# morisUtokyo/mTR

Measured on AMD Instinct MI355X. Metric: reads/sec, 2 kb Nanopore synthetic, higher is better.
Workload: dtype int32

## Files before the change

### mtr_amd/csrc/device_util.hip.inc

```
#pragma once
#include <hip/hip_runtime.h>
#include "mtr_common.h"
#include "walk_screen.h"

#define DEVINL __device__ __forceinline__

typedef __attribute__((address_space(3))) int lds_int;
typedef __attribute__((address_space(3))) unsigned char lds_u8;

DEVINL int lane_id() { return (int)(threadIdx.x & 63u); }
__device__ long long mtr_dev_wrap_dp_size = MTRC_WRAP_DP_SIZE;
DEVINL bool dp_size_ok(int U, int rows) { return (size_t)(U + 1) * (size_t)rows + (size_t)U < (size_t)mtr_dev_wrap_dp_size; }
DEVINL int uni(int v) { return __builtin_amdgcn_readfirstlane(v); }
DEVINL long long uni64(long long v)
{
    const unsigned lo = (unsigned)__builtin_amdgcn_readfirstlane((int)(unsigned)v);
    const unsigned hi = (unsigned)__builtin_amdgcn_readfirstlane((int)(unsigned)((unsigned long long)v >> 32));
    return (long long)(((unsigned long long)hi << 32) | lo);
}
DEVINL int bcast(int v, int src) { return __shfl(v, src, 64); }
DEVINL unsigned long long lanemask_lt() { return (1ull << lane_id()) - 1ull; }
DEVINL int mbcnt(unsigned long long m)
{
    return (int)__builtin_amdgcn_mbcnt_hi((unsigned)(m >> 32), __builtin_amdgcn_mbcnt_lo((unsigned)m, 0u));
}
DEVINL int first_lane(unsigned long long m) { return __ffsll((long long)m) - 1; }


DEVINL unsigned scan_max_u32(unsigned v);
DEVINL int wave_max_i32(int v)
{
    for (int d = 32; d > 0; d >>= 1) { int o = __shfl_xor(v, d, 64); v = o > v ? o : v; }
    return v;
}
DEVINL int lane_val(int v, int l) { return __builtin_amdgcn_readlane(v, l); }
DEVINL int write_lane(int v, int val, int l)
{
    asm("s_mov_b32 m0, %2\n\tv_writelane_b32 %0, %1, m0" : "+v"(v) : "s"(val), "s"(l) : "m0");
    return v;
}
DEVINL void write_lane2(int &a, int &b, int va, int vb, int l)
{
    asm("s_mov_b32 m0, %4\n\tv_writelane_b32 %0, %2, m0\n\tv_writelane_b32 %1, %3, m0" : "+v"(a), "+v"(b) : "s"(va), "s"(vb), "s"(l & 63) : "m0");
}
DEVINL long long lane_val64(long long v, int l)
{
    const unsigned lo = (unsigned)__builtin_amdgcn_readlane((int)(unsigned)v, l), hi = (unsigned)__builtin_amdgcn_readlane((int)(unsigned)((unsigned long long)v >> 32), l);
    return (long long)(((unsigned long long)hi << 32) | lo);
}
DEVINL int wave_max_i32_dpp(int v) { return lane_val((int)scan_max_u32((unsigned)(v + 1)), 63) - 1; }
DEVINL long long wave_sum_i64(long long v)
{
    for (int d = 32; d > 0; d >>= 1) v += __shfl_xor(v, d, 64);
    return v;
}

DEVINL unsigned scan_max_u32(unsigned v)
{
    unsigned t;
    t = (unsigned)__builtin_amdgcn_update_dpp(0, (int)v, 0x111, 0xf, 0xf, false); v = t > v ? t : v;
    t = (unsigned)__builtin_amdgcn_update_dpp(0, (int)v, 0x112, 0xf, 0xf, false); v = t > v ? t : v;
    t = (unsigned)__builtin_amdgcn_update_dpp(0, (int)v, 0x114, 0xf, 0xf, false); v = t > v ? t : v;
    t = (unsigned)__builtin_amdgcn_update_dpp(0, (int)v, 0x118, 0xf, 0xf, false); v = t > v ? t : v;
    t = (unsigned)__builtin_amdgcn_update_dpp(0, (int)v, 0x142, 0xa, 0xf, false); v = t > v ? t : v;
    t = (unsigned)__builtin_amdgcn_update_dpp(0, (int)v, 0x143, 0xc, 0xf, false); v = t > v ? t : v;
    return v;
}
DEVINL void scan_max_u32_x2(unsigned &a, unsigned &b)
{
    unsigned s, t;
#define MTR_SCAN_STEP(ctrl, rm) \
    s = (unsigned)__builtin_amdgcn_update_dpp(0, (int)a, ctrl, rm, 0xf, false); \
    t = (unsigned)__builtin_amdgcn_update_dpp(0, (int)b, ctrl, rm, 0xf, false); \
    a = s > a ? s : a; b = t > b ? t : b;
    MTR_SCAN_STEP(0x111, 0xf) MTR_SCAN_STEP(0x112, 0xf) MTR_SCAN_STEP(0x114, 0xf) MTR_SCAN_STEP(0x118, 0xf)
    MTR_SCAN_STEP(0x142, 0xa) MTR_SCAN_STEP(0x143, 0xc)
#undef MTR_SCAN_STEP
}
DEVINL void scan_max_u32_x2_row16(unsigned &a, unsigned &b)
{
    unsigned s, t;
#define MTR_SCAN_STEP(ctrl) \
    s = (unsigned)__builtin_amdgcn_update_dpp(0, (int)a, ctrl, 0xf, 0xf, false); \
    t = (unsigned)__builtin_amdgcn_update_dpp(0, (int)b, ctrl, 0xf, 0xf, false); \
    a = s > a ? s : a; b = t > b ? t : b;
    MTR_SCAN_STEP(0x111) MTR_SCAN_STEP(0x112) MTR_SCAN_STEP(0x114) MTR_SCAN_STEP(0x118)
#undef MTR_SCAN_STEP
}
DEVINL int row_shift_up1(int v, int first)
{
    return __builtin_amdgcn_update_dpp(first, v, 0x111, 0xf, 0xf, false);
}
typedef unsigned short u16x2 __attribute__((ext_vector_type(2)));
DEVINL u16x2 as_pk(unsigned v) { return __builtin_bit_cast(u16x2, v); }
DEVINL unsigned as_u32(u16x2 v) { return __builtin_bit_cast(unsigned, v); }
DEVINL unsigned pk_add(unsigned a, unsigned b) { return as_u32(as_pk(a) + as_pk(b)); }
DEVINL unsigned pk_sub(unsigned a, unsigned b) { return as_u32(as_pk(a) - as_pk(b)); }
DEVINL unsigned pk_sub_sat(unsigned a, unsigned b) { return as_u32(__builtin_elementwise_sub_sat(as_pk(a), as_pk(b))); }
DEVINL unsigned max3_u32(unsigned a, unsigned b, unsigned c) { unsigned r; asm("v_max3_u32 %0, %1, %2, %3" : "=v"(r) : "v"(a), "v"(b), "v"(c)); return r; }
DEVINL unsigned pk_max(unsigned a, unsigned b) { return as_u32(__builtin_elementwise_max(as_pk(a), as_pk(b))); }
DEVINL unsigned pk_min(unsigned a, unsigned b) { return as_u32(__builtin_elementwise_min(as_pk(a), as_pk(b))); }
template <int SH>
DEVINL unsigned lshl_or(unsigned a, unsigned b)
{
    unsigned r;
    asm("v_lshl_or_b32 %0, %1, %2, %3" : "=v"(r) : "v"(a), "n"(SH), "v"(b));
    return r;
}
DEVINL unsigned pk_nonzero(unsigned a, unsigned one_pk)
{
    unsigned r;
    asm("v_pk_min_u16 %0, %1, %2" : "=v"(r) : "v"(a), "v"(one_pk));
    return r;
}

DEVINL int shift_up1(int v, int first)
{
    return __builtin_amdgcn_update_dpp(first, v, 0x138, 0xf, 0xf, false);
}

DEVINL void scan_max_first(double &v, int &idx)
{
    int lane = lane_id();
    for (int d = 1; d < 64; d <<= 1) {
        double ov = __shfl_up(v, d, 64); int oi = __shfl_up(idx, d, 64);
        if (lane >= d && !(v > ov)) { v = ov; idx = oi; }
    }
}
DEVINL void scan_min_first(double &v, int &idx)
{
    int lane = lane_id();
    for (int d = 1; d < 64; d <<= 1) {
        double ov = __shfl_up(v, d, 64); int oi = __shfl_up(idx, d, 64);
        if (lane >= d && !(v < ov)) { v = ov; idx = oi; }
    }
}
// ... 134 lines not shown
```

### mtr_amd/csrc/dp_test.hip.inc

```
#pragma once
#include "dp_wrap.hip.inc"

struct DpPassArgs {
    DpTestArgs t;
    int32_t pass, n_groups;
    const int32_t *group_off;
    long long packed_words;
};

DEVINL void dpt_clear(DpRes &o) { o.stop_i = 0; o.end_i = 0; o.mat = o.mis = o.ins = o.del = o.scanned = 0; o.end_j = 0; }
DEVINL void dpt_store(const DpPassArgs &a, int task, int p, int qs, int U, const DpRes &o)
{
    if (lane_id() == 0) {
        int32_t *r = a.t.out8 + ((size_t)task * 2 + (size_t)p) * 8;
        r[0] = qs + o.stop_i + 1; r[1] = qs + o.end_i; r[2] = o.end_i - o.stop_i; r[3] = U > 0 ? o.scanned / U : 0;
        r[4] = o.mat; r[5] = o.mis; r[6] = o.ins; r[7] = o.del;
    }
}
template <int FMT>
DEVINL void dpt_traceback(const DpPassArgs &a, const uint32_t *pk, int qs, int U, const uint8_t *cells, int psel, int rstride, const int (&best)[3],
                          DpRes &o, unsigned long long *wc)
{
    dpt_clear(o);
    const int bv = uni(best[0]), bi = uni(best[1]), bj = uni(best[2]);
// ... 125 lines not shown
        }
        const int maxrows = uni(wave_max_i32(q.rows)), umax = uni(wave_max_i32(q.U));
        const int C = (umax + 7) >> 3;
        int best[2][3];
        st_fwd2p_oct(C, q, cells, maxrows, best);
        wave_sync_mem();
        const int bestl = st_oct_best_lanes(best);
#pragma unroll 1
        for (int g = 0; g < n; g++) {
            const int tg = t0 + g;
            const int rd = uni(a.t.read_idx[tg]), qs = uni(a.t.qs[tg]), U = uni(a.t.unit_off[tg + 1]) - uni(a.t.unit_off[tg]);
            for (int p = 0; p < 2; p++) {
                const int bk[3] = { lane_val(bestl, 8 * g + 3 * p), lane_val(bestl, 8 * g + 3 * p + 1), lane_val(bestl, 8 * g + 3 * p + 2) };
                DpRes o;
                dpt_traceback<1>(a, a.t.b.packed + uni64(a.t.b.woff[rd]), qs, U, cells + (size_t)g * DPQ_DP_BYTES_G(8, C, maxrows), p, DPQ_ROW_BYTES_G(8, C), bk, o, s_cnt);
                dpt_store(a, tg, p, qs, U, o);
                loop_join();
            }
            loop_join();
        }
        wave_sync_mem();
        loop_join();
    }
    wc_flush(s_cnt, a.t.counters);
}

__global__ __launch_bounds__(64, MTR_WAVES_PER_SIMD) void mtr_k_dp_test_rev(DpPassArgs a)
{
    __shared__ unsigned long long s_cnt[CNT_N];
    if (lane_id() < CNT_N) s_cnt[lane_id()] = 0ull;
    uint8_t *cells = a.t.scratch + (size_t)blockIdx.x * a.t.scratch_per_wave;
    for (;;) {
        const int grp = next_work_item(a.t.work_counter);
        if (grp >= a.n_groups) break;
        const int t0 = uni(a.group_off[grp]), n = uni(a.group_off[grp + 1]) - t0;
        DpOct q; q.n = n;
        int maxrows = 0, maxU = 0;
#pragma unroll 1
        for (int g = 0; g < RQ_SLOTS; g++) { q.pk[g] = a.t.b.packed; q.wlim[g] = 1; q.base[g] = 0; q.rows[g] = 0; q.U[g] = 0; q.unit[g] = cells; q.G[g] = 1; q.MM[g] = 1; q.D[g] = 1; }
#pragma unroll 1
        for (int k = 0; k < n; k++) {
            const int tg = t0 + k;
            const int rd = uni(a.t.read_idx[tg]), uo = uni(a.t.unit_off[tg]);
            q.pk[k] = a.t.b.packed + uni64(a.t.b.woff[rd]); q.wlim[k] = a.packed_words - uni64(a.t.b.woff[rd]);
            q.base[k] = uni(a.t.qs[tg]); q.rows[k] = uni(a.t.qe[tg]) - q.base[k] + 1;
            q.U[k] = uni(a.t.unit_off[tg + 1]) - uo; q.unit[k] = a.t.units + uo;
            q.G[k] = uni(a.t.gain[tg]); q.MM[k] = uni(a.t.mism[tg]); q.D[k] = uni(a.t.indel[tg]);
            maxrows = q.rows[k] > maxrows ? q.rows[k] : maxrows; maxU = q.U[k] > maxU ? q.U[k] : maxU;
        }
        const int Cq = DPQ_COLS(maxU);
        int best[RQ_SLOTS][3];
        for (int g = 0; g < RQ_SLOTS; g++) { best[g][0] = 0; best[g][1] = 0; best[g][2] = 0; }
        if (a.pass == MTR_TEST_PASS_FOUR1P) st_fwd1p_four(Cq, q, cells, maxrows, best); else st_fwd1p_any(Cq, q, cells, maxrows, best);
        wave_sync_mem();
#pragma unroll 1
        for (int k = 0; k < n; k++) {
            int bk[3] = { best[0][0], best[0][1], best[0][2] };
#pragma unroll
            for (int h = 1; h < RQ_SLOTS; h++) if (k == h) { bk[0] = best[h][0]; bk[1] = best[h][1]; bk[2] = best[h][2]; }
            const int tg = t0 + k;
            const int rd = uni(a.t.read_idx[tg]), qs = uni(a.t.qs[tg]), U = uni(a.t.unit_off[tg + 1]) - uni(a.t.unit_off[tg]);
            DpRes o;
            dpt_traceback<3>(a, a.t.b.packed + uni64(a.t.b.woff[rd]), qs, U, cells + (size_t)k * DPQP_DP_BYTES(Cq, maxrows), 0, DPQ_ROW_BYTES(Cq), bk, o, s_cnt);
            dpt_store(a, tg, 0, qs, U, o);
            loop_join();
        }
        wave_sync_mem();
        loop_join();
    }
    wc_flush(s_cnt, a.t.counters);
}

struct PolishTestArgs {
    K2Args a;
    int32_t n_tasks;
    const int32_t *read_idx, *rep_start, *rep_end, *k;
    const uint8_t *units; const int32_t *scores, *unit_off;
    uint8_t *out_units; int32_t *out_len;
};
__global__ __launch_bounds__(64, MTR_LAT_WAVES_PER_SIMD) void mtr_k_polish_test(PolishTestArgs p)
{
    __shared__ __attribute__((aligned(16))) int s_arena[MTR_ARENA_INTS];
    __shared__ unsigned long long s_cnt[CNT_N];
    int *s_keys = s_arena, *s_seeds = s_arena + K2_TAB_CAP, *s_stage = s_seeds + MTRC_MAX_SEEDS + 4;
    const int lane = lane_id();
    if (lane < CNT_N) s_cnt[lane] = 0ull;
    K2Ctx c;
    c.a = &p.a; c.wc = s_cnt;
    c.sc = p.a.scratch + (size_t)blockIdx.x * p.a.scratch_per_wave;
    c.y = k2_layout(p.a.Lmax, p.a.cells_cap);
    c.lds_keys = (lds_int *)s_keys; c.seeds = (lds_int *)s_seeds; c.stage = (lds_int *)s_stage;
    c.ties = (int *)(c.sc + c.y.ties); c.fresh = c.ties + MTRC_MAX_TIEBREAKS;
    c.memo_n = 0; c.memo_qs = c.memo_qe = -1; c.memo_U = 0; c.rmemo_n = 0;
    for (;;) {
        const int t = next_work_item(p.a.work_counter);
        if (t >= p.n_tasks) break;
        st_member_ctx(c, p.a, uni(p.read_idx[t]));
        const int uo = uni(p.unit_off[t]), U = uni(p.unit_off[t + 1]) - uo;
        RR r; rr_clear(r);
        r.rep_start = uni(p.rep_start[t]); r.rep_end = uni(p.rep_end[t]); r.kmer = uni(p.k[t]); r.period = U;
        uint8_t *ub = slot_unit(c, 1);
        slot_load_candidate(ub, slot_score(c, 1), p.units + uo, p.scores + uo, U);
        wave_sync_mem();
        polish(c, r, 1);
#pragma unroll 1
        for (int q = lane; q < r.period; q += 64) p.out_units[(size_t)t * MTRC_MAX_PERIOD + q] = ub[q];
        if (lane == 0) p.out_len[t] = r.period;
        wave_sync_mem();
        loop_join();
    }
    wc_flush(s_cnt, p.a.counters);
}

struct ReviseTestArgs {
    K2Args a;
    int32_t n_groups;
    const int32_t *group_off, *read_idx, *rr;
    const uint8_t *units; const int32_t *scores, *unit_off;
    int32_t *out_rr; uint8_t *out_units;
};
__global__ __launch_bounds__(64, MTR_WAVES_PER_SIMD) void mtr_k_revise_test(ReviseTestArgs p)
{
    __shared__ __attribute__((aligned(16))) int s_arena[MTR_ARENA_INTS];
    __shared__ unsigned long long s_cnt[CNT_N];
    int *s_keys = s_arena, *s_seeds = s_arena + K2_TAB_CAP, *s_stage = s_seeds + MTRC_MAX_SEEDS + 4;
    const int lane = lane_id();
    if (lane < CNT_N) s_cnt[lane] = 0ull;
    K2Ctx c;
    c.a = &p.a; c.wc = s_cnt;
    c.sc = p.a.scratch + (size_t)blockIdx.x * p.a.scratch_per_wave;
    c.y = k2_layout(p.a.Lmax, p.a.cells_cap);
    c.lds_keys = (lds_int *)s_keys; c.seeds = (lds_int *)s_seeds; c.stage = (lds_int *)s_stage;
    c.ties = (int *)(c.sc + c.y.ties); c.fresh = c.ties + MTRC_MAX_TIEBREAKS;
    for (;;) {
        const int grp = next_work_item(p.a.work_counter);
        if (grp >= p.n_groups) break;
        const int t0 = uni(p.group_off[grp]), t1 = uni(p.group_off[grp + 1]);
        c.memo_n = 0; c.memo_qs = c.memo_qe = -1; c.memo_U = 0; c.rmemo_n = 0;
#pragma unroll 1
        for (int t = t0; t < t1; t++) {
            st_member_ctx(c, p.a, uni(p.read_idx[t]));
            const int uo = uni(p.unit_off[t]), U = uni(p.unit_off[t + 1]) - uo;
            RR cur; st_rr_load(p.rr + (size_t)t * 13, cur);
            uint8_t *ub = slot_unit(c, 1);
            slot_load_candidate(ub, slot_score(c, 1), p.units + uo, p.scores + uo, U);
            wave_sync_mem();
            revise(c, cur);
            if (lane == 0) {
                int32_t *o = p.out_rr + (size_t)t * 13;
                o[0] = cur.rep_start; o[1] = cur.rep_end; o[2] = cur.repeat_len; o[3] = cur.period; o[4] = cur.copies; o[5] = cur.mat; o[6] = cur.mis;
                o[7] = cur.ins; o[8] = cur.del; o[9] = cur.kmer; o[10] = cur.G; o[11] = cur.MM; o[12] = cur.D;
            }
#pragma unroll 1
            for (int q = lane; q < cur.period && q < MTRC_MAX_PERIOD; q += 64) p.out_units[(size_t)t * MTRC_MAX_PERIOD + q] = ub[q];
            wave_sync_mem();
            loop_join();
        }
        loop_join();
    }
    wc_flush(s_cnt, p.a.counters);
}
```

### mtr_amd/csrc/k1_ranges.hip.inc

```
#pragma once
#include "device_util.hip.inc"


struct K1Pass { int k, w; };
typedef short k1_num;
static_assert(2 * MTRC_MAX_WINDOW <= 32767, "numerators in 16 bits");

DEVINL int k1_raw(const uint32_t *pk, const uint8_t *mt, int L, int r, int N, int idx)
{
    if (idx < r) return mt[N + idx];
    if (idx < r + L) return base_at(pk, idx - r);
    if (idx < L + 2 * r) return mt[N + r + (idx - r - L)];
    if (idx < N) return mt[idx];
    return 0;
}
DEVINL int k1_raw_tail(const uint32_t *pk, const uint8_t *mt, int L, int r, int N, int idx, const uint16_t *tail, int E, int tlen)
{
    if (idx >= E) return idx - E < tlen ? (int)tail[idx - E] : 0;
    return k1_raw(pk, mt, L, r, N, idx);
}

template <bool MANHATTAN>
DEVINL void k1_passes(const K1Layout &y, uint8_t *sc, unsigned short *hist, int hist_cap, int L, int r, int npass, int pass_k, int pass_w,
                      int32_t *status, int row_base = 0, int alloc_nb = 0)
// ... 1063 lines not shown
    }
    double *DI = (double *)(sc + y.di); int *END = (int *)(sc + y.end); int *W = (int *)(sc + y.w);
    if (parts & K1_CODES) for (int idx = lane; idx < n; idx += 64) DI[idx] = -1.0;
    wave_sync_mem();

    const bool rows_hold_d = MANHATTAN && (parts & K1_PASSES) && (parts & K1_FINISH) && only_pass < 0 && seg < 0 && !(MAY_FILE_ORDER && tlen > 0) && 2 * n <= arena_bytes;
    if (npass > 0 && (parts & K1_PASSES)) {
        const unsigned long long t_p = clk();
        int run_n = npass, run_k = my_k, run_w = my_w, row_base = 0;
        if (only_pass >= 0) {
            run_n = only_pass < npass ? 1 : 0; row_base = only_pass;
            run_k = __shfl(my_k, only_pass & 63, 64); run_w = __shfl(my_w, only_pass & 63, 64);
        }
        if (run_n > 0) {
            if (seg > 0 && MAY_FILE_ORDER && tlen > 0) {  }
            else if (seg >= 0 && !(MAY_FILE_ORDER && tlen > 0)) {
                if (MANHATTAN) k1_passes_manhattan(y, sc, arena, arena_bytes, L, r, 1, run_k, run_w, a.status, row_base, seg);
                else k1_pass_pearson_seg(y, sc, arena, L, r, run_k, run_w, only_pass, seg);
            }
            else if (MAY_FILE_ORDER && tlen > 0) k1_passes<MANHATTAN>(y, sc, (unsigned short *)arena, arena_bytes / 2, L, r, run_n, run_k, run_w, a.status, row_base, 1024);
            else if (MANHATTAN) k1_passes_manhattan(y, sc, arena, arena_bytes, L, r, run_n, run_k, run_w, a.status, row_base, -1, !rows_hold_d);
            else k1_passes<false>(y, sc, (unsigned short *)arena, arena_bytes / 2, L, r, run_n, run_k, run_w, a.status, row_base);
        }
        wc_time(wc, CYC_K1_PASSES, t_p);
    }
    if (!(parts & K1_FINISH)) return;
    if (npass > 0) {
        const unsigned long long t_e = clk();
        const double *tmp = (const double *)(sc + y.tmp);
        if (!(parts & K1_NO_EXTRACT))
        for (int p = 0; p < npass; p++) {
            int w = __shfl(my_w, p, 64);
            if (MANHATTAN) {
                const k1_num *row = (const k1_num *)(sc + y.tmp) + (size_t)p * n;
                if (2 * n <= arena_bytes) {
                    lds_i16 *r16 = (lds_i16 *)arena;
                    const int bits_at = (2 * n + 3) & ~3, bits_words = (n + 31) >> 5;
                    const bool bits = bits_at + 4 * bits_words <= arena_bytes;
                    lds_u32b *pres = (lds_u32b *)(arena + bits_at);
                    if (bits && p == 0) { for (int t = lane; t < bits_words; t += 64) pres[t] = 0u; }
                    if (rows_hold_d) {
                        const int ns = n - w - r - __shfl(my_k, p, 64) + 1;
                        for (int t = lane; t < n; t += 64) r16[t] = (short)((ns > 0 && t >= w && t < w + ns) ? (int)row[t - w] - (int)row[t] : -2 * w);
                    } else
                    for (int t = lane; t < n; t += 64) r16[t] = (short)row[t];
                    wave_sync_mem();
                    if (bits) k1_extract_int<true, true>(row, r16, n, w, DI, END, W, wc, pres); else k1_extract_int<true>(row, r16, n, w, DI, END, W, wc);
                    wave_sync_mem();
                } else k1_extract_int<false>(row, nullptr, n, w, DI, END, W, wc);
            }
            else k1_extract(tmp + (size_t)p * n, n, w, DI, END, W, wc);
        }
        wc_time(wc, CYC_K1_EXTRACT, t_e);
        wc_add(wc, CNT_DI_PASSES, npass);
        long long pos = (lane < npass) ? (long long)(n - my_w - r - my_k + 1) : 0; if (pos < 0) pos = 0;
        pos = wave_sum_i64(pos);
        wc_add(wc, CNT_DI_POS, pos);
    }

    const unsigned long long t_d = clk();
    int alive_n = 0;
    for (int base = 0; base < L; base += 64) {
        const int i = base + lane;
        alive_n += __popcll(__ballot(i < L && DI[i + r] != -1.0));
    }
    int nout;
    if ((alive_n + 1) * 20 <= arena_bytes) {
        lds_f64 *ld = (lds_f64 *)arena;
        lds_i32 *lp = (lds_i32 *)(arena + 8 * (alive_n + 1)), *le = lp + (alive_n + 1), *lw = le + (alive_n + 1);
        nout = k1_lists(a, rd, L, r, DI, END, W, lp, le, lw, ld, alive_n + 1);
    } else {
        int *lp = (int *)(sc + y.l_pos), *le = (int *)(sc + y.l_end), *lw = (int *)(sc + y.l_w);
        double *ld = (double *)(sc + y.l_di);
        nout = k1_lists(a, rd, L, r, DI, END, W, lp, le, lw, ld, y.cap);
    }
    const int ocap = mtrc_range_cap(L);
    if (nout > ocap) { set_status(a.status, DEV_ERR_RANGE_OVERFLOW); nout = ocap; }
    if (lane == 0) a.r_count[rd] = nout;
    wc_add(wc, CNT_RANGES_CAND, nout);
    wc_time(wc, CYC_K1_DEDUP, t_d);
    wc_time(wc, CYC_K1_TOTAL, t_start);
}

#define MTR_ARENA_INTS (2048 + 104 + 256)

__global__ __launch_bounds__(64, 4) void mtr_k1_part(K1Args a, int parts, const int32_t *item_read, const int32_t *item_pass, int n_items)
{
    __shared__ __attribute__((aligned(16))) int s_arena[MTR_ARENA_INTS];
    __shared__ unsigned long long s_cnt[CNT_N];
    if (lane_id() < CNT_N) s_cnt[lane_id()] = 0ull;
    for (;;) {
        const int t = next_work_item(a.work_counter);
        if (t >= n_items) break;
        const int rd = item_read ? __builtin_amdgcn_readfirstlane(item_read[t]) : t;
        const int pv = item_pass ? __builtin_amdgcn_readfirstlane(item_pass[t]) : -1;
        const int ps = pv < 0 ? -1 : (pv & 255), seg = pv < 0 ? -1 : (pv >> 8) - 1;
        uint8_t *sc = a.scratch + (size_t)rd * a.scratch_per_wave;
        if (a.manhattan) k1_read<true, true>(a, rd, sc, (lds_u8 *)s_arena, MTR_ARENA_INTS * 4, s_cnt, parts, ps, seg);
        else k1_read<false, true>(a, rd, sc, (lds_u8 *)s_arena, MTR_ARENA_INTS * 4, s_cnt, parts, ps, seg);
        loop_join();
    }
    wc_flush(s_cnt, a.counters);
}

#define K1_PIPE_ARENA_BYTES (K1_PIPE_WAVES * K1_TILE * 16)
__global__ __launch_bounds__(64 * K1_PIPE_WAVES) void mtr_k1_finish_pipe(K1Args a, int n_items, int seg_rows )
{
    __shared__ __attribute__((aligned(16))) int s_arena[K1_PIPE_ARENA_BYTES / 4];
    __shared__ unsigned long long s_cnt[K1_PIPE_WAVES][CNT_N];
    __shared__ int s_progress[MTRC_MAX_PASSES + 1];
    __shared__ int s_wg[2 * K1_PIPE_WAVES + 2];
    __shared__ int s_item;
#ifdef MTR_K1_COUNT
    __shared__ unsigned long long s_dbg[MTRC_MAX_PASSES + 1][5];
#endif
    const int wv = threadIdx.x >> 6, lane = lane_id();
    if (lane < CNT_N) s_cnt[wv][lane] = 0ull;
    for (;;) {
        __syncthreads();
        if (threadIdx.x == 0) s_item = (int)atomicAdd(a.work_counter, 1u);
        if (threadIdx.x < MTRC_MAX_PASSES + 1) s_progress[threadIdx.x] = 0;
        __syncthreads();
        const int rd = __builtin_amdgcn_readfirstlane(s_item);
        if (rd >= n_items) break;
        uint8_t *sc = a.scratch + (size_t)rd * a.scratch_per_wave;
        const int L = a.b.lens[rd];
        const int r = mtrc_rand_len(L);
        const int n = L + 2 * r;
        const K1Layout y = k1_layout(a.Lmax);
        double *DI = (double *)(sc + y.di); int *END = (int *)(sc + y.end); int *W = (int *)(sc + y.w);
        int npass = 0;
        for (int k = 1; k <= 5; k += 2) {
            const int max_w = (k == 1) ? 20 : (k == 3 ? 80 : MTRC_MAX_WINDOW);
            for (int w = MTRC_MIN_WINDOW; w <= max_w && w < L / 2; w *= 2) npass++;
        }
#ifdef MTR_K1_COUNT
        const unsigned long long tk0 = __builtin_amdgcn_s_memtime();
#endif
        for (int p = wv; p < npass; p += K1_PIPE_WAVES) {
            int w = 0, kk = 1, q = 0;
            for (int k = 1; k <= 5; k += 2) {
                const int max_w = (k == 1) ? 20 : (k == 3 ? 80 : MTRC_MAX_WINDOW);
                for (int ww = MTRC_MIN_WINDOW; ww <= max_w && ww < L / 2; ww *= 2) { if (q == p) { w = ww; kk = k; } q++; }
            }
            if (a.manhattan && seg_rows) { k1_numerators(y, sc, L, r, kk, w, p); wave_sync_mem(); }
            K1Pipe pp;
            pp.prev = p > 0 ? (volatile lds_i32 *)&s_progress[p - 1] : nullptr;
            pp.mine = (volatile lds_i32 *)&s_progress[p];
            lds_u8 *mine = (lds_u8 *)s_arena + (size_t)wv * (K1_TILE * 16);
            if (a.manhattan) {
                K1Tile<int, k1_num> tl; tl.val = (lds_i32 *)(mine + K1_TILE * 8); tl.di = (lds_f64 *)mine;
                tl.row = (const k1_num *)(sc + y.tmp) + (size_t)p * n; tl.DI = DI; tl.n = n; tl.t0 = 0; tl.tn = 0; tl.pad = 0; tl.pp = pp;
#ifdef MTR_K1_COUNT
                const unsigned long long tp0 = __builtin_amdgcn_s_memtime();
#endif
                k1_extract_int_tile(tl, n, w, DI, END, W, s_cnt[wv]);
#ifdef MTR_K1_COUNT
                if (lane == 0) { s_dbg[p][0] = tp0 - tk0; s_dbg[p][1] = __builtin_amdgcn_s_memtime() - tk0; s_dbg[p][2] = tl.c_wait; s_dbg[p][3] = tl.c_fill;
                                 s_dbg[p][4] = (unsigned long long)tl.n_rec | ((unsigned long long)tl.n_refill << 32); }
#endif
            } else {
                K1Tile<double> tl; tl.val = (lds_f64 *)(mine + K1_TILE * 8); tl.di = (lds_f64 *)mine;
                tl.row = (const double *)(sc + y.tmp) + (size_t)p * n; tl.DI = DI; tl.n = n; tl.t0 = 0; tl.tn = 0; tl.pad = 0.0; tl.pp = pp;
                k1_extract_tile(tl, n, w, DI, END, W);
            }
            wave_sync_mem();
            if (lane == 0) s_progress[p] = 0x7fffffff;
            loop_join();
        }
        __syncthreads();
#ifdef MTR_K1_COUNT
        const unsigned long long tk1 = __builtin_amdgcn_s_memtime();
#endif
        {
#ifdef MTR_K1_COUNT
            int nout = k1_lists_wg(a, rd, L, r, y, sc, (lds_u8 *)s_arena, K1_PIPE_ARENA_BYTES, (volatile lds_i32 *)s_wg, s_dbg[20]);
#else
            int nout = k1_lists_wg(a, rd, L, r, y, sc, (lds_u8 *)s_arena, K1_PIPE_ARENA_BYTES, (volatile lds_i32 *)s_wg);
#endif
            if (wv == 0) {
                const int ocap = mtrc_range_cap(L);
                if (nout > ocap) { set_status(a.status, DEV_ERR_RANGE_OVERFLOW); nout = ocap; }
                if (lane == 0) a.r_count[rd] = nout;
                wc_add(s_cnt[0], CNT_RANGES_CAND, nout);
                wc_add(s_cnt[0], CNT_DI_PASSES, npass);
                long long pos = 0;
                { int q = 0; for (int k = 1; k <= 5; k += 2) { const int max_w = (k == 1) ? 20 : (k == 3 ? 80 : MTRC_MAX_WINDOW);
                    for (int ww = MTRC_MIN_WINDOW; ww <= max_w && ww < L / 2; ww *= 2) { const long long t = (long long)n - ww - r - k + 1; if (t > 0) pos += t; q++; } } }
                wc_add(s_cnt[0], CNT_DI_POS, pos);
            }
        }
#ifdef MTR_K1_COUNT
        __syncthreads();
        if (threadIdx.x == 0) {
            const unsigned long long tk2 = __builtin_amdgcn_s_memtime();
            for (int p = 0; p < npass; p++) printf("pass %2d: start %7.3f end %7.3f Mcyc  wait %7.3f fill %7.3f  rec %5d refills %5d\n", p, (double)s_dbg[p][0] * 1e-6, (double)s_dbg[p][1] * 1e-6,
                                                   (double)s_dbg[p][2] * 1e-6, (double)s_dbg[p][3] * 1e-6, (int)(s_dbg[p][4] & 0xffffffffu), (int)(s_dbg[p][4] >> 32));
            printf("read %d: extraction %7.3f Mcyc, phase D %7.3f Mcyc (compaction+cuts %7.3f, chain %7.3f)\n", rd, (double)(tk1 - tk0) * 1e-6, (double)(tk2 - tk1) * 1e-6,
                   (double)s_dbg[20][0] * 1e-6, (double)s_dbg[20][1] * 1e-6);
        }
#endif
    }
    wc_flush(s_cnt[wv], a.counters);
}

__global__ __launch_bounds__(64, 4) void mtr_k1_ranges(K1Args a)
{
    __shared__ __attribute__((aligned(16))) int s_arena[MTR_ARENA_INTS];
    __shared__ unsigned long long s_cnt[CNT_N];
    if (lane_id() < CNT_N) s_cnt[lane_id()] = 0ull;
    uint8_t *sc = a.scratch + (size_t)blockIdx.x * a.scratch_per_wave;
    for (;;) {
        const int t = next_work_item(a.work_counter);
        if (t >= a.b.n_reads) break;
        int rd = a.b.order[t];
        if (a.manhattan) k1_read<true, true>(a, rd, sc, (lds_u8 *)s_arena, MTR_ARENA_INTS * 4, s_cnt);
        else k1_read<false, true>(a, rd, sc, (lds_u8 *)s_arena, MTR_ARENA_INTS * 4, s_cnt);
        loop_join();
    }
    wc_flush(s_cnt, a.counters);
}
```

### mtr_amd/csrc/k2_units.hip.inc

```
#pragma once
#include "device_util.hip.inc"
#include "dp_wrap.hip.inc"
#include "min_missing_table.h"
#include "polish_plan.h"

#ifndef MTR_WAVES_PER_SIMD
#define MTR_WAVES_PER_SIMD 4
#endif
#ifndef MTR_LAT_WAVES_PER_SIMD
#define MTR_LAT_WAVES_PER_SIMD 5
#endif
#define MTR_LDS_PER_CU (160 * 1024)
#define MTR_LDS_GRANULE 1280
#define MTR_LDS_ALLOC(bytes) (((bytes) + MTR_LDS_GRANULE - 1) / MTR_LDS_GRANULE * MTR_LDS_GRANULE)
#define MTR_ARENA_CORESIDENT_BYTES (7 * MTR_LDS_GRANULE)
#define K2_TAB_CAP 2048
#define K2_TAB_MAX_WIDTH 1400
#define K2_EMPTY (-1)

__device__ __constant__ char d_min_missing[2001] = MTR_MIN_MISSING_DIGITS_STR;

struct RR {
    int rep_start, rep_end, repeat_len, period, copies, mat, mis, ins, del, kmer, G, MM, D;
};
// ... 299 lines not shown
                unsigned bk = tab_bucket(t, key);
                bool done = false;
                for (unsigned n = 0; n <= t.mask && !done; n++) {
                    for (int sl = 0; sl < 4 && !done; sl++) {
                        const unsigned at = 4 * bk + (unsigned)sl;
                        int seen;
                        if (t.use_lds) {
                            int expected = K2_EMPTY;
                            bool won = __hip_atomic_compare_exchange_strong(&c.lds_keys[at], &expected, key, __ATOMIC_RELAXED, __ATOMIC_RELAXED, __HIP_MEMORY_SCOPE_WORKGROUP);
                            seen = won ? key : expected;
                        } else {
                            int prev = atomicCAS(&t.gkeys[at], K2_EMPTY, key);
                            seen = prev == K2_EMPTY ? key : prev;
                        }
                        if (seen == key) {
                            if (t.vals_lds) {
                                const int nv = __hip_atomic_fetch_add(&c.lds_keys[K2_VALS_LDS_OFF + at], 1, __ATOMIC_RELAXED, __HIP_MEMORY_SCOPE_WORKGROUP) + 1;
                                mx = nv > mx ? nv : mx;
                            } else {
                                (void)__hip_atomic_fetch_add(&t.gvals[at], 1, __ATOMIC_RELAXED, __HIP_MEMORY_SCOPE_AGENT);
                            }
                            done = true;
                        }
                    }
                    bk = (bk + 1) & t.mask;
                }
            }
        }
    }
    wave_sync_mem();
    if (t.fmt == TAB_SPLIT && !t.vals_lds) {
        for (unsigned base = 0; base < cap; base += 512) {
            int v[8];
#pragma unroll
            for (int q = 0; q < 8; q++) { const unsigned sidx = base + 64u * (unsigned)q + (unsigned)lane; v[q] = sidx < cap ? __hip_atomic_load(&t.gvals[sidx], __ATOMIC_RELAXED, __HIP_MEMORY_SCOPE_AGENT) : 0; }
#pragma unroll
            for (int q = 0; q < 8; q++) mx = v[q] > mx ? v[q] : mx;
        }
    }
    t.n_compact = -1; t.ckeys = (int *)(c.sc + c.y.ckeys); t.cslots = (int *)(c.sc + c.y.cslots);
    if (!t.use_lds && t.fmt == TAB_SPLIT) {
        int nc = 0;
        for (unsigned base = 0; base < cap; base += 512) {
            int kq[8];
#pragma unroll
            for (int q = 0; q < 8; q++) { const unsigned sidx = base + 64u * (unsigned)q + (unsigned)lane; kq[q] = sidx < cap ? t.gkeys[sidx] : K2_EMPTY; }
#pragma unroll
            for (int q = 0; q < 8; q++) {
                const unsigned sidx = base + 64u * (unsigned)q + (unsigned)lane;
                const int key = kq[q];
                const unsigned long long m = __ballot(key != K2_EMPTY);
                if (key != K2_EMPTY) { const int at = nc + mbcnt(m); t.ckeys[at] = key; t.cslots[at] = (int)sidx; }
                nc += __popcll(m);
            }
        }
        t.n_compact = nc;
        wave_sync_mem();
    }
    c.tab = t; c.tab_k = k;
    {
        c.tab_gen++;
        const int nsc = t.use_lds ? K2_STEP_CACHE_LDS : K2_STEP_CACHE;
        const int bit = t.use_lds ? 1 : 3;
        if ((c.sc_ready & bit) != bit) {
            int4 *sc_ = (int4 *)(c.sc + c.y.step_cache);
            for (int q = lane; q < 2 * nsc; q += 64) sc_[q] = make_int4(-1, 0, 0, 0);
            c.sc_ready |= bit;
            wave_sync_mem();
        }
    }
    wc_add(c.wc, CNT_TABLES, 1);
    mx = wave_max_i32_dpp(mx);
    wc_time(c.wc, CYC_TAB_BUILD, t0);
#ifdef MTR_PROFILE_WALK_FMT
    if (MTR_PROFILE_WALK_FMT >= 4) {
        const int cls_ = t.fmt == TAB_DIRECT ? (k <= 4 ? CNT_SPARE43 : CNT_SPARE44) : t.fmt == TAB_PACKED ? (t.nslots <= 1024u ? CNT_SPARE45 : CNT_SPARE46)
                         : t.use_lds ? CNT_SPARE47 : CNT_SPARE55;
        if (MTR_PROFILE_WALK_FMT == 4) wc_time(c.wc, cls_, t0); else wc_add(c.wc, cls_, 1);
    }
#endif
    return mx;
}

DEVINL int tab_seeds(K2Ctx &c, int k, int qs, int qe, int max_freq)
{
    const int lane = lane_id();
    const unsigned long long t0 = clk();
    int n = 0;
    for (int base = qs; base <= qe && n < MTRC_MAX_SEEDS; base += 64) {
        int i = base + lane;
        int key = 0; bool cand = false;
        if (i <= qe) { key = win_node(c.pk, c.L, k, qe, i); cand = (tab_get(c, key) == max_freq); }
        unsigned long long m = __ballot(cand);
        while (m != 0ull && n < MTRC_MAX_SEEDS) {
            int t = first_lane(m);
            int sk = lane_val(key, t);
            if (lane == 0) { c.seeds[n] = sk; tab_dec(c, sk); }
            n++;
            m &= ~__ballot(cand && key == sk);
            m &= ~(1ull << t);
            loop_join();
        }
        loop_join();
    }
    wave_sync_mem();
    wc_time(c.wc, CYC_SEEDS, t0);
    return n;
}

DEVINL unsigned rev_pairs(unsigned x)
{
    x = __brev(x);
    return ((x >> 1) & 0x55555555u) | ((x & 0x55555555u) << 1);
}

DEVINL unsigned rev_digits(unsigned x, int e)
{
    if (e <= 0) return 0u;
    unsigned r = __brev(x);
    r = ((r >> 1) & 0x55555555u) | ((r & 0x55555555u) << 1);
    return r >> (32 - 2 * e);
}

#define K2_IDX_MIN_KEYS 512
DEVINL unsigned idx_bucket(bool backward, unsigned key, int k)
{
    return backward ? rev_digits(key & 1023u, 5) : (key >> (2 * k - 10));
}
DEVINL void idx_build(K2Ctx &c, bool backward, int k)
{
    const int lane = lane_id();
    const Tab &t = c.tab;
    const int n = t.n_compact;
    lds_int *ends = c.lds_keys + (backward ? 1024 : 0);
    int *gk = (int *)(c.sc + (backward ? c.y.gkb : c.y.gkf)), *gs = (int *)(c.sc + (backward ? c.y.gsb : c.y.gsf));
    for (int b = lane; b < 1024; b += 64) ends[b] = 0;
    __builtin_amdgcn_fence(__ATOMIC_RELEASE, "workgroup"); __builtin_amdgcn_wave_barrier();
    for (int base = 0; base < n; base += 512) {
        int kq[8];
#pragma unroll
        for (int q = 0; q < 8; q++) { const int i = base + 64 * q + lane; kq[q] = i < n ? t.ckeys[i] : K2_EMPTY; }
#pragma unroll
        for (int q = 0; q < 8; q++) if (kq[q] != K2_EMPTY) (void)__hip_atomic_fetch_add(&ends[idx_bucket(backward, (unsigned)kq[q], k)], 1, __ATOMIC_RELAXED, __HIP_MEMORY_SCOPE_WORKGROUP);
    }
    __builtin_amdgcn_fence(__ATOMIC_ACQ_REL, "workgroup"); __builtin_amdgcn_wave_barrier();
    {
        int cnt[16], sum = 0;
#pragma unroll
        for (int q = 0; q < 16; q++) { cnt[q] = ends[16 * lane + q]; sum += cnt[q]; }
        int incl = sum;
        for (int d = 1; d < 64; d <<= 1) { const int o = __shfl_up(incl, d, 64); if (lane >= d) incl += o; }
        int run = incl - sum;
#pragma unroll
        for (int q = 0; q < 16; q++) { ends[16 * lane + q] = run; run += cnt[q]; }
    }
    __builtin_amdgcn_fence(__ATOMIC_ACQ_REL, "workgroup"); __builtin_amdgcn_wave_barrier();
    for (int base = 0; base < n; base += 512) {
        int kq[8], sq[8];
#pragma unroll
        for (int q = 0; q < 8; q++) { const int i = base + 64 * q + lane; kq[q] = i < n ? t.ckeys[i] : K2_EMPTY; sq[q] = i < n ? t.cslots[i] : 0; }
#pragma unroll
        for (int q = 0; q < 8; q++) if (kq[q] != K2_EMPTY) {
            const int at = __hip_atomic_fetch_add(&ends[idx_bucket(backward, (unsigned)kq[q], k)], 1, __ATOMIC_RELAXED, __HIP_MEMORY_SCOPE_WORKGROUP);
            gk[at] = kq[q]; gs[at] = sq[q];
        }
    }
    wave_sync_mem();
    if (backward) c.idx_gen_b = c.tab_gen; else c.idx_gen_f = c.tab_gen;
}
DEVINL void idx_range(const K2Ctx &c, bool backward, unsigned fixed, int f, int &lo, int &hi)
{
    const lds_int *ends = c.lds_keys + (backward ? 1024 : 0);
    unsigned blo, bhi;
    if (f >= 5) { blo = backward ? rev_digits(fixed & 1023u, 5) : (fixed >> (2 * (f - 5))); bhi = blo; }
    else {
        const unsigned r = backward ? rev_digits(fixed, f) : fixed;
        blo = r << (2 * (5 - f)); bhi = ((r + 1u) << (2 * (5 - f))) - 1u;
    }
    lo = blo == 0u ? 0 : uni(ends[blo - 1u]);
    hi = uni(ends[bhi]);
}

DEVINL int lookahead(K2Ctx &c, bool backward, int node, int k, int look, int &m_exit, long long &lookups)
{
    const int lane = lane_id();
    const Tab &t = c.tab;
    const unsigned cap = t.nslots;
    {
        const int s1 = k - 1;
        int cnt1 = -1;
        if (lane < 4) {
            const int cand = !backward ? (((node & ((1 << (2 * s1)) - 1)) << 2) + lane) : ((lane << (2 * s1)) + (node >> 2));
            cnt1 = tab_get(c, cand);
        }
        const int c0 = lane_val(cnt1, 0), c1 = lane_val(cnt1, 1), c2 = lane_val(cnt1, 2), c3 = lane_val(cnt1, 3);
        int bst = c0, first = 0;
        if (c1 > bst) { bst = c1; first = 1; }
        if (c2 > bst) { bst = c2; first = 2; }
        if (c3 > bst) { bst = c3; first = 3; }
        const int nf1 = (c0 == bst ? 1 : 0) + (c1 == bst ? 1 : 0) + (c2 == bst ? 1 : 0) + (c3 == bst ? 1 : 0);
        wc_add(c.wc, CNT_WALK_STEPS, 1);
        if (nf1 == 1 || look == 1) { lookups += 4; m_exit = nf1 == 1 ? 1 : 2; return first; }
    }
    wc_add(c.wc, CNT_WALK_SLOW, 1);
    const unsigned long long t_slow = clk();
    const bool grouped = t.n_compact >= K2_IDX_MIN_KEYS && k >= 5;
    if (grouped && (backward ? c.idx_gen_b : c.idx_gen_f) != c.tab_gen) idx_build(c, backward, k);
    const int *gk = (const int *)(c.sc + (backward ? c.y.gkb : c.y.gkf)), *gs = (const int *)(c.sc + (backward ? c.y.gsb : c.y.gsf));
    int *B = c.ties, *Bn = c.fresh;
    int nb = 1, e = 0, m0 = 0;
    int breg = 0;
    int best_digit = 0;
    int m;
    for (m = 1; m <= look; m++) {
        const int nt = (e >= 5 || (nb << (2 * e)) >= MTRC_MAX_TIEBREAKS) ? MTRC_MAX_TIEBREAKS : (nb << (2 * e));
        const int ncand = 4 * nt;
        const int s = k - m;
        const int fixed = backward ? (node >> (2 * m)) : (node & ((1 << (2 * s)) - 1));
        const int emask = (1 << (2 * e)) - 1;
        int best = -1, nf = 0;
        best_digit = 0;
        bool evaluated = false;
        if (m == 2 && m0 == 0 && e == 1 && look > 2) {
            const int top = look < 12 ? look : 12;
            unsigned hits = 0u;
            const unsigned kmask = (k >= 16) ? 0xffffffffu : ((1u << (2 * k)) - 1u);
            unsigned lvN[11], lvT[11];
#pragma unroll
            for (int mm = 2; mm <= 12; mm++) {
                const int wbits = 2 * (k - mm) + (mm > 6 ? 2 * (mm - 6) : 0);
                if (!backward) { lvN[mm - 2] = ((unsigned)node << (2 * (mm < 16 ? mm : 15))) & kmask; lvT[mm - 2] = (1u << (mm < 6 ? 2 * mm : 12)) - 1u; }
                else { lvN[mm - 2] = mm <= top ? __builtin_bitreverse32((unsigned)node >> (2 * mm)) : 0u; lvT[mm - 2] = (mm > top || wbits <= 0) ? 0xffffffffu : ((1u << (32 - wbits)) - 1u); }
            }
            const bool compact = t.n_compact >= 0;
            const unsigned nscan = compact ? (unsigned)t.n_compact : cap;
            if (grouped) {
                for (int mm = 2; mm <= top && hits == 0u; mm++) {
                    const int f = k - mm;
                    const unsigned fx = backward ? ((unsigned)node >> (2 * mm)) : ((unsigned)node & ((1u << (2 * f)) - 1u));
                    int lo, hi;
                    idx_range(c, backward, fx, f, lo, hi);
                    const int wb = 2 * f + (mm > 6 ? 2 * (mm - 6) : 0);
                    const unsigned gN = !backward ? (((unsigned)node << (2 * mm)) & kmask) : __builtin_bitreverse32((unsigned)node >> (2 * mm));
                    const unsigned gT = !backward ? ((1u << (mm < 6 ? 2 * mm : 12)) - 1u) : (wb <= 0 ? 0xffffffffu : ((1u << (32 - wb)) - 1u));
                    for (int base = lo; base < hi; base += 64) {
                        const int i = base + lane;
                        const int keyi = i < hi ? gk[i] : K2_EMPTY;
                        const unsigned x = backward ? __builtin_bitreverse32((unsigned)keyi) : (unsigned)keyi;
                        if (__ballot(keyi != K2_EMPTY && (x ^ gN) <= gT) != 0ull) { hits = 1u << (mm - 2); break; }
                    }
                    lookups += hi - lo;
                }
            } else
            for (unsigned base = 0; base < nscan; base += 64) {
                const unsigned sidx = base + (unsigned)lane;
                int keyi = K2_EMPTY, cnti = 0;
                if (sidx < nscan) { if (compact) keyi = t.ckeys[sidx]; else tab_slot(c, sidx, keyi, cnti); }
                const unsigned x = backward ? __builtin_bitreverse32((unsigned)keyi) : (unsigned)keyi;
                unsigned h = 0u, tmp;
#pragma unroll
                for (int mm = 12; mm >= 2; mm--)
                    asm("v_xor_b32 %1, %2, %3\n\tv_cmp_ge_u32 vcc, %4, %1\n\tv_addc_co_u32 %0, vcc, %0, %0, vcc" : "+v"(h), "=&v"(tmp) : "s"(lvN[mm - 2]), "v"(x), "s"(lvT[mm - 2]) : "vcc");
                if (keyi != K2_EMPTY) hits |= h;
            }
            hits &= (1u << (top - 1)) - 1u;
            int first_hit = top + 1;
            for (int mm = top; mm >= 2; mm--) if (__ballot((hits >> (mm - 2)) & 1u) != 0ull) first_hit = mm;
            if (!grouped) lookups += nscan;
            if (first_hit > 2) {
                if (first_hit > look) {
                    m = look + 1; best_digit = 0;
                    break;
                }
                e = first_hit - 1; m = first_hit - 1;
                continue;
            }
        }
        if (nb <= 64 && ncand >= 128 && (unsigned)ncand * 4u > (t.n_compact >= 0 ? (unsigned)t.n_compact : cap)) {
            int nmatch = 0;
            const bool compact = t.n_compact >= 0;
            unsigned nscan = compact ? (unsigned)t.n_compact : cap, scan0 = 0u;
            const int *sk = t.ckeys, *ss = t.cslots;
            if (grouped) {
                int lo, hi;
                idx_range(c, backward, (unsigned)fixed, s, lo, hi);
                scan0 = (unsigned)lo; nscan = (unsigned)hi; sk = gk; ss = gs;
            }
            for (unsigned base = scan0; base < nscan; base += 64) {
                const unsigned sidx = base + (unsigned)lane;
                int key = K2_EMPTY, scnt = 0;
                if (sidx < nscan) { if (compact) key = sk[sidx]; else tab_slot(c, sidx, key, scnt); }
                bool hit = key != K2_EMPTY;
                int d = 0;
                if (!backward) { hit = hit && ((key >> (2 * m)) == fixed); d = key & ((1 << (2 * m)) - 1); }
                else { hit = hit && ((key & ((1 << (2 * s)) - 1)) == fixed); d = (int)((unsigned)key >> (2 * s)); }
                int b, x, j;
                if (!backward) { j = d & 3; x = (d >> 2) & emask; b = d >> (2 * (e + 1)); }
                else { b = d & ((1 << (2 * m0)) - 1); j = d >> (2 * (m0 + e)); x = (int)rev_digits((unsigned)((d >> (2 * m0)) & emask), e); }
                int bi = -1;
                for (int q = 0; q < nb; q++) { const int bv = lane_val(breg, q); if (bv == b) bi = q; }
                const long long ti = bi < 0 ? -1 : (((long long)bi) << (2 * e)) + x;
                hit = hit && bi >= 0 && ti < MTRC_MAX_TIEBREAKS;
                const int idx = (int)ti * 4 + j;
                if (compact && hit) scnt = t.gvals[ss[sidx]];
                const int cnt = hit ? scnt : -1;
                const unsigned long long hm = __ballot(hit);
                if (hm != 0ull) {
                    const int pos = nmatch + mbcnt(hm);
                    if (hit && pos < 64) { c.stage[pos] = cnt; c.stage[64 + pos] = idx; c.stage[128 + pos] = d; }
                    nmatch += __popcll(hm);
                }
                loop_join();
            }
            lookups += nscan - scan0;
            if (nmatch <= 64) {
                evaluated = true;
                if (nmatch == 0) {
                    best = 0; nf = ncand < MTRC_MAX_TIEBREAKS ? ncand : MTRC_MAX_TIEBREAKS;
                    const int b0 = lane_val(breg, 0);
                    best_digit = backward ? b0 : (b0 << (2 * (e + 1)));
                } else {
                    __builtin_amdgcn_wave_barrier();
                    const bool mine = lane < nmatch;
                    const int cnt = mine ? c.stage[lane] : -1, idx = mine ? c.stage[64 + lane] : 0x7fffffff, d = mine ? c.stage[128 + lane] : 0;
                    best = wave_max_i32_dpp(cnt);
                    const bool tie = mine && cnt == best;
                    int rank = 0;
                    for (int q = 0; q < nmatch; q++) {
                        const int iq = lane_val(idx, q), cq = lane_val(cnt, q);
                        if (cq == best && iq < idx) rank++;
                    }
                    const unsigned long long tm = __ballot(tie);
                    nf = __popcll(tm);
                    if (tie) c.stage[192 + rank] = d;
                    __builtin_amdgcn_wave_barrier();
                    best_digit = uni(c.stage[192]);
                }
            }
        }
        if (!evaluated) {
            best = -1; nf = 0; best_digit = 0;
            const int p4m1 = 1 << (2 * (m - 1));
            for (int base = 0; base < ncand; base += 64) {
                const int ci = base + lane;
                int cnt = -1, digit = 0;
                const int ti = ci >> 2, j = ci & 3, bi = ti >> (2 * e), x = ti & emask;
                const int bshfl = __shfl(breg, bi & 63, 64);
                if (ci < ncand) {
                    const int bval = (m0 == 0) ? 0 : (nb <= 64 ? bshfl : B[bi]);
                    int cand;
                    if (!backward) { const int tv = (bval << (2 * e)) | x; digit = 4 * tv + j; cand = ((node & ((1 << (2 * s)) - 1)) << (2 * m)) + digit; }
                    else { const int tv = bval + (int)(rev_digits((unsigned)x, e) << (2 * m0)); digit = j * p4m1 + tv; cand = (digit << (2 * s)) + (node >> (2 * m)); }
                    cnt = tab_get(c, cand);
                }
                const int cm = wave_max_i32_dpp(cnt);
                if (cm > best) { best = cm; nf = 0; }
                const unsigned long long eq = __ballot(ci < ncand && cnt == best);
                if (eq != 0ull) {
                    if (nf == 0) best_digit = lane_val(digit, first_lane(eq));
                    const int pos = nf + mbcnt(eq);
                    if (cnt == best && ci < ncand && pos < MTRC_MAX_TIEBREAKS) { if (pos < 64) c.stage[192 + pos] = digit; else Bn[pos] = digit; }
                    nf += __popcll(eq); if (nf > MTRC_MAX_TIEBREAKS) nf = MTRC_MAX_TIEBREAKS;
                }
                loop_join();
            }
            lookups += ncand;
        }
        if (nf <= 1) break;
        if (best == 0) {
            e += 1;
        } else {
            __builtin_amdgcn_wave_barrier();
            nb = nf; e = 0; m0 = m;
            breg = lane < nb ? c.stage[192 + lane] : 0;
            if (nb > 64) { Bn[lane] = breg; wave_sync_mem(); int *sw = B; B = Bn; Bn = sw; }
        }
        loop_join();
    }
    m_exit = m;
    wc_time(c.wc, CYC_WALK_SLOW, t_slow);
    return best_digit;
}

struct WalkState { int node, l, pend, pend_at, status, fast_steps, chk_node, chk_l, chk_pow; };
enum { WALK_RUNNING = 0, WALK_CLOSED = 1, WALK_CYCLE = 2 };
DEVINL bool walk_cycle_check(int node, int l, int &chk_node, int &chk_l, int &chk_pow)
{
    if (node == chk_node) return true;
    if (l - chk_l >= chk_pow) { chk_node = node; chk_l = l; chk_pow *= 2; }
    return false;
}

typedef __attribute__((address_space(1))) uint8_t glb_u8;
typedef __attribute__((address_space(1))) int glb_int;
#define TAB_SPLIT_GLOBAL 3
template <int FMT, bool BACKWARD, bool EARLY>
DEVINL void walk_pair_steps(lds_int *keys, const Tab &t, uint8_t *ub_, int *us_, int k, int seed, int max_steps, WalkState &w)
{
    const int lane = lane_id();
    glb_u8 *ub = (glb_u8 *)ub_; glb_int *us = (glb_int *)us_;
    const int sh1 = 2 * (k - 1), p4k1 = 1 << sh1, m1 = p4k1 - 1;
    const unsigned kmask = (1u << (2 * k)) - 1u;
    const int q = lane - 4, jj = (q >> 2) & 3, cc = q & 3;
    const bool lvl1 = lane < 4, lvl2 = lane >= 4 && lane < 20;
    const bool active = lane < (BACKWARD ? 20 : 21);
    const int l_sh = lvl1 ? 2 : lvl2 ? 4 : 0;
    const int l_add = BACKWARD ? (lvl1 ? (lane << sh1) : lvl2 ? ((cc << sh1) + (jj << (sh1 - 2))) : 0)
                               : (lvl1 ? lane : lvl2 ? ((jj << 2) + cc) : 0);
    int node = w.node, l = w.l, pend = w.pend, status = WALK_RUNNING;
    const int l_in = l;
    int chk_node = w.chk_node, chk_l = w.chk_l, chk_pow = w.chk_pow;
    int lo = l, ubuf = 0, sbuf = 0;
    auto flush = [&](int hi) {
        const int li = (lo & ~63) + lane;
        if (li >= lo && li < hi) { ub[li] = (uint8_t)ubuf; if (li > 0) us[li - 1] = sbuf; }
    };
    int done = 0;
    while (l < max_steps) {
        const unsigned key = BACKWARD ? ((unsigned)node >> l_sh) + (unsigned)l_add : ((((unsigned)node << l_sh) & kmask) + (unsigned)l_add);
        int cnt = -1;
        bool more = false;
        if (FMT == TAB_DIRECT) {
            const unsigned wd = (unsigned)keys[key >> 1];
            const int cv = (int)((wd >> (16 * (key & 1u))) & 0xffffu);
            cnt = active ? (key < t.nslots ? cv : 0) : -1;
        } else if (FMT == TAB_PACKED) {
            const unsigned b0 = (tab_hash((int)key) >> 9) & t.mask, b1 = (b0 + 1u) & t.mask;
            const v4i ka = *(const lds_v4i *)(keys + 4 * b0), kb = *(const lds_v4i *)(keys + 4 * b1);
            auto rot = [&](int wv) { const unsigned d = (unsigned)wv ^ key; return (unsigned)__builtin_amdgcn_alignbit(d, d, K2_PACK_KEY_BITS); };
            auto min3u = [](unsigned x, unsigned y, unsigned z) { const unsigned m = x < y ? x : y; return m < z ? m : z; };
            const unsigned mn = min3u(min3u(rot(ka.x), rot(ka.y), rot(ka.z)), min3u(rot(ka.w), rot(kb.x), rot(kb.y)), min3u(rot(kb.z), rot(kb.w), 0xffffffffu));
            const bool present = mn < 4095u;
            more = active && !present && ka.w != K2_EMPTY && kb.w != K2_EMPTY;
            cnt = active ? (present ? (int)mn : 0) : -1;
        }
        if (FMT == TAB_SPLIT || FMT == TAB_SPLIT_GLOBAL) {
            const unsigned b0 = tab_bucket(t, (int)key), b1 = (b0 + 1u) & t.mask;
            v4i ka, kb;
            if (FMT == TAB_SPLIT) { ka = *(const lds_v4i *)(keys + 4 * b0); kb = *(const lds_v4i *)(keys + 4 * b1); }
            else if (active) { ka = *(const v4i *)(t.gkeys + 4 * b0); kb = *(const v4i *)(t.gkeys + 4 * b1); }
            else { ka = kb = (v4i){ K2_EMPTY, K2_EMPTY, K2_EMPTY, K2_EMPTY }; }
            const int ik = (int)key;
            int idx = kb.w == ik ? (int)(4u * b1 + 3u) : -1;
            idx = kb.z == ik ? (int)(4u * b1 + 2u) : idx; idx = kb.y == ik ? (int)(4u * b1 + 1u) : idx; idx = kb.x == ik ? (int)(4u * b1) : idx;
            idx = ka.w == ik ? (int)(4u * b0 + 3u) : idx; idx = ka.z == ik ? (int)(4u * b0 + 2u) : idx;
            idx = ka.y == ik ? (int)(4u * b0 + 1u) : idx; idx = ka.x == ik ? (int)(4u * b0) : idx;
            const bool present = active && idx >= 0;
            more = active && idx < 0 && ka.w != K2_EMPTY && kb.w != K2_EMPTY;
            int cv = 0;
            if (present) cv = (FMT == TAB_SPLIT && t.vals_lds) ? keys[K2_VALS_LDS_OFF + idx] : t.gvals[idx];
            cnt = active ? cv : -1;
        }
        const unsigned more_m = FMT != TAB_DIRECT ? (unsigned)__ballot(more) : 0u;
        if (FMT != TAB_DIRECT && (more_m & (BACKWARD ? 0xfu : 0x10000fu)) != 0u) {
            if (more && (lane < 4 || lane == 20)) cnt = tab_get_raw<(FMT == TAB_SPLIT_GLOBAL ? TAB_SPLIT : FMT)>(keys, t, (int)key);
        }
        int qmax; unsigned eqm;
// ... 58 lines not shown
    t.gkeys = (int *)uni64((long long)gkeys); t.gvals = (int *)uni64((long long)gvals);
    t.n_compact = -1; t.ckeys = nullptr; t.cslots = nullptr;
    WalkState w;
    w.node = uni(node); w.l = uni(l); w.pend = uni(pend); w.pend_at = uni(pend_at); w.status = WALK_RUNNING; w.fast_steps = 0;
    w.chk_node = uni(chk_node); w.chk_l = uni(chk_l); w.chk_pow = uni(chk_pow);
    {
        int nfast = 0;
#define WALK_PAIR(EARLY_, LIM_) do { \
            if (t.fmt == TAB_DIRECT) { if (backward) walk_pair_steps<TAB_DIRECT, true, EARLY_>(keys, t, ub, us, k, seed, LIM_, w); else walk_pair_steps<TAB_DIRECT, false, EARLY_>(keys, t, ub, us, k, seed, LIM_, w); } \
            else if (t.fmt == TAB_PACKED) { if (backward) walk_pair_steps<TAB_PACKED, true, EARLY_>(keys, t, ub, us, k, seed, LIM_, w); else walk_pair_steps<TAB_PACKED, false, EARLY_>(keys, t, ub, us, k, seed, LIM_, w); } \
            else if (t.use_lds) { if (backward) walk_pair_steps<TAB_SPLIT, true, EARLY_>(keys, t, ub, us, k, seed, LIM_, w); else walk_pair_steps<TAB_SPLIT, false, EARLY_>(keys, t, ub, us, k, seed, LIM_, w); } \
            else { if (backward) walk_pair_steps<TAB_SPLIT_GLOBAL, true, EARLY_>(keys, t, ub, us, k, seed, LIM_, w); else walk_pair_steps<TAB_SPLIT_GLOBAL, false, EARLY_>(keys, t, ub, us, k, seed, LIM_, w); } } while (0)
        if (w.l < 10) {
            const int lim = max_steps < 10 ? max_steps : 10;
            WALK_PAIR(true, lim);
            nfast = w.fast_steps;
        }
        if (w.status == WALK_RUNNING && w.l >= 10 && w.l < max_steps) {
            WALK_PAIR(false, max_steps);
            nfast += w.fast_steps;
        }
#undef WALK_PAIR
        w.fast_steps = nfast;
    }
    return w;
}

#define MTRC_SCREEN_MIN_SEEDS 8
template <int FMT, bool BACKWARD>
DEVINL int walk_screen_steps(lds_int *keys, const Tab &t, int k, int seed, bool active, int max_steps)
{
    const int sh1 = 2 * (k - 1), p4k1 = 1 << sh1, m1 = p4k1 - 1;
    int node = seed, res = 0;
    bool run = active;
    int chk_node = -1, chk_l = -1, chk_pow = 1;
    for (int l = 0; l < max_steps; l++) {
        const unsigned long long m_run = __ballot(run), m_pos = __ballot(res != 0);
        if (m_run == 0ull) break;
        if (m_pos != 0ull && (m_run & ((1ull << first_lane(m_pos)) - 1ull)) == 0ull) break;
        if (run) {
            int cnt[4]; bool more[4];
#pragma unroll
            for (int j = 0; j < 4; j++) cnt[j] = tab_get_first<FMT>(keys, t, BACKWARD ? ((j << sh1) + (node >> 2)) : (((node & m1) << 2) + j), more[j]);
            if (more[0] || more[1] || more[2] || more[3]) {
#pragma unroll
                for (int j = 0; j < 4; j++) if (more[j]) cnt[j] = tab_get_raw<FMT>(keys, t, BACKWARD ? ((j << sh1) + (node >> 2)) : (((node & m1) << 2) + j));
            }
            int bst = cnt[0], first = 0;
            if (cnt[1] > bst) { bst = cnt[1]; first = 1; }
            if (cnt[2] > bst) { bst = cnt[2]; first = 2; }
            if (cnt[3] > bst) { bst = cnt[3]; first = 3; }
            const int nf1 = (cnt[0] == bst ? 1 : 0) + (cnt[1] == bst ? 1 : 0) + (cnt[2] == bst ? 1 : 0) + (cnt[3] == bst ? 1 : 0);
            if (nf1 != 1 && l >= 10) { res = 2; run = false; }
            else {
                node = BACKWARD ? (first * p4k1 + (node >> 2)) : (4 * (node & m1) + (nf1 == 1 ? first : 0));
                if (node == seed) { res = (l + 1 < MTRC_MAX_PERIOD) ? 1 : 0; run = false; }
                else if (l >= 10 && walk_cycle_check(node, l, chk_node, chk_l, chk_pow)) { res = 0; run = false; }
            }
        }
        loop_join();
    }
    return res;
}
__device__ __attribute__((noinline)) int walk_screen(lds_int *keys, Tab t, int k, int seed, int active, int max_steps, int backward)
{
    keys = (lds_int *)(unsigned)uni((int)(unsigned)(unsigned long long)keys);
    k = uni(k); max_steps = uni(max_steps); backward = uni(backward);
    t.fmt = uni(t.fmt); t.use_lds = uni(t.use_lds); t.vals_lds = uni(t.vals_lds); t.mask = (unsigned)uni((int)t.mask); t.nslots = (unsigned)uni((int)t.nslots);
    t.gkeys = (int *)uni64((long long)t.gkeys); t.gvals = (int *)uni64((long long)t.gvals);
    const bool act = active != 0;
    if (t.fmt == TAB_DIRECT) return backward ? walk_screen_steps<TAB_DIRECT, true>(keys, t, k, seed, act, max_steps) : walk_screen_steps<TAB_DIRECT, false>(keys, t, k, seed, act, max_steps);
    if (t.fmt == TAB_PACKED) return backward ? walk_screen_steps<TAB_PACKED, true>(keys, t, k, seed, act, max_steps) : walk_screen_steps<TAB_PACKED, false>(keys, t, k, seed, act, max_steps);
    return backward ? walk_screen_steps<TAB_SPLIT, true>(keys, t, k, seed, act, max_steps) : walk_screen_steps<TAB_SPLIT, false>(keys, t, k, seed, act, max_steps);
}
DEVINL int screen_seeds(K2Ctx &c, bool backward, int qs, int qe, int k, int s, int ns)
{
    const int lane = lane_id();
    int max_steps = (qe - qs) / MTRC_MIN_NUM_FREQ_UNIT; if (max_steps > MTRC_MAX_PERIOD) max_steps = MTRC_MAX_PERIOD;
    const unsigned long long t0 = clk();
    int first = ns;
    for (int b = s; b < ns && first == ns; b += 64) {
        const int idx = b + lane;
        const bool act = idx < ns;
        const int sd = act ? (int)c.seeds[idx] : 0;
        const int r = walk_screen(c.lds_keys, c.tab, k, sd, act ? 1 : 0, max_steps, backward ? 1 : 0);
        const unsigned long long m = __ballot(act && r != 0);
        if (m != 0ull) first = b + first_lane(m);
        loop_join();
    }
    wc_time(c.wc, CYC_WALK, t0);
    return uni(first);
}

DEVINL int walk(K2Ctx &c, bool backward, int qs, int qe, int k, int seed, int dst)
{
    const int lane = lane_id();
    uint8_t *ub = slot_unit(c, dst); int *us = slot_score(c, dst);
    const int p4k1 = 1 << (2 * (k - 1));
    int period = 0;
    const unsigned long long t0 = clk();
    int max_steps = (qe - qs) / MTRC_MIN_NUM_FREQ_UNIT; if (max_steps > MTRC_MAX_PERIOD) max_steps = MTRC_MAX_PERIOD;
    long long lookups = 0;
    WalkState w; w.node = seed; w.l = 0; w.pend = 0; w.pend_at = -1; w.status = WALK_RUNNING; w.fast_steps = 0;
    w.chk_node = -1; w.chk_l = -1; w.chk_pow = 1;
    wc_add(c.wc, CNT_WALK_CALLS, 1);
    while (w.l < max_steps) {
        const unsigned long long t_fast = clk();
        w = walk_fast(c.lds_keys, c.tab.fmt, c.tab.use_lds, c.tab.vals_lds, c.tab.mask, c.tab.nslots, c.tab.gkeys, c.tab.gvals, ub, us, k, seed, max_steps, backward ? 1 : 0,
                      w.node, w.l, w.pend, w.pend_at, w.chk_node, w.chk_l, w.chk_pow);
        wc_time(c.wc, CYC_WALK_FAST, t_fast);
#ifdef MTR_PROFILE_WALK_FMT
        if (c.prof_kernel == 1 && MTR_PROFILE_WALK_FMT <= 3) {
            const Tab &pt = c.tab;
            const int cls_ = pt.fmt == TAB_DIRECT ? CNT_SPARE43 : pt.fmt == TAB_PACKED ? (pt.nslots <= 1024u ? CNT_SPARE44 : CNT_SPARE45)
                             : !pt.use_lds ? CNT_SPARE55 : pt.vals_lds ? CNT_SPARE46 : CNT_SPARE47;
            if (MTR_PROFILE_WALK_FMT == 1) wc_time(c.wc, cls_, t_fast);
            else if (MTR_PROFILE_WALK_FMT == 2) wc_add(c.wc, cls_, uni(w.fast_steps));
            else wc_add(c.wc, cls_, 1);
        }
#endif
        const int l = uni(w.l);
        int node = uni(w.node), pend_score = uni(w.pend), pend_at = uni(w.pend_at);
        const int status = uni(w.status);
        lookups += 4ll * uni(w.fast_steps);
        wc_add(c.wc, CNT_WALK_STEPS, uni(w.fast_steps));
        if (status == WALK_CLOSED) { period = l + 1; if (MTRC_MAX_PERIOD <= period) period = 0; break; }
        if (status == WALK_CYCLE || l >= max_steps) break;
        if (!backward) {
            if (lane == 0 && l > 0) us[l - 1] = pend_score;
            pend_score = uni(tab_get(c, node));
            if (lane == 0) ub[l] = (uint8_t)(node >> (2 * (k - 1)));
            pend_at = l;
        }
        const int nsc = c.tab.use_lds ? K2_STEP_CACHE_LDS : K2_STEP_CACHE;
        int4 *sce = (int4 *)(c.sc + c.y.step_cache) + ((backward ? nsc : 0) + (int)((tab_hash(node) >> 7) & (unsigned)(nsc - 1)));
        const int from = node;
        const int4 ce = *sce;
        const int ck = uni(ce.x), cv = uni(ce.y), cg = uni(ce.z);
        if (ck == from && cg == c.tab_gen) {
            node = cv;
            if (backward) {
                if (lane == 0 && l > 0) us[l - 1] = pend_score;
                pend_score = uni(tab_get(c, node));
                if (lane == 0) ub[l] = (uint8_t)(node >> (2 * (k - 1)));
                pend_at = l;
            }
        } else {
        int m;
        const int best_digit = lookahead(c, backward, node, k, k, m, lookups);
        if (!backward) node = 4 * (node & (p4k1 - 1)) + (m - 1 >= 15 ? 0 : (best_digit >> (2 * (m - 1))));
        else {
            node = (best_digit & 3) * p4k1 + (node >> 2);
            if (lane == 0 && l > 0) us[l - 1] = pend_score;
            pend_score = uni(tab_get(c, node));
            if (lane == 0) ub[l] = (uint8_t)(node >> (2 * (k - 1)));
            pend_at = l;
        }
        if (lane == 0) *sce = make_int4(from, node, c.tab_gen, 0);
        wave_sync_mem();
        }
        w.node = node; w.l = l + 1; w.pend = pend_score; w.pend_at = pend_at;
        loop_join();
        if (node == seed) { period = l + 1; if (MTRC_MAX_PERIOD <= period) period = 0; break; }
        {
            int cn = uni(w.chk_node), cl = uni(w.chk_l), cp = uni(w.chk_pow);
            const bool cyc = walk_cycle_check(node, l, cn, cl, cp);
            w.chk_node = cn; w.chk_l = cl; w.chk_pow = cp;
// ... 154 lines not shown
    int best[4][2][3];
    const unsigned long long t_f = clk();
    dp_forward2p_q4(c.pk, qs, rows, q, 1, 1, 3, 1, 3, 1, codes, best);
    wave_sync_mem();
    wc_time(c.wc, CYC_DP_FWD, t_f);
    wc_time_aux(c.wc, CNT_SPARE47, t_f);
    const unsigned long long t_b = clk();
#pragma unroll
    for (int g = 0; g < 4; g++) {
        if (g < n) {
            const int U = q.U[g];
            RR r; rr_clear(r); r.period = U; r.kmer = kk[g];
            RR bestr; rr_clear(bestr);
            float best_ratio = -1.0f;
            long long tb = 0;
            bool ok = true;
            for (int p = 0; p < 2; p++) {
                DpRes o; o.stop_i = 0; o.end_i = 0; o.mat = o.mis = o.ins = o.del = o.scanned = 0; o.end_j = 0;
                const int bv = uni(best[g][p][0]), bi = uni(best[g][p][1]), bj = uni(best[g][p][2]);
                if (bv > 0) {
                    dp_traceback<0, 1>(c.pk, qs, U, codes + q.off[g], p, U, bi, bj, nullptr, nullptr, nullptr, o, c.wc);
                    if (o.stop_i < 0) { o.stop_i = 0; o.end_i = 0; o.mat = o.mis = o.ins = o.del = o.scanned = 0; ok = false; }
                }
                tb += (long long)(o.mat + o.mis + o.ins + o.del);
                RR t = r;
                apply_dp(t, qs, o, U, 1, p == 0 ? 1 : 3, p == 0 ? 3 : 1);
                trace_ev(c, 3, qs, qe, U, trace_on(c, 3) ? unit_hash(q.unit[g], U) : 0, 1, p == 0 ? 1 : 3, p == 0 ? 3 : 1, t.rep_start, t.rep_end, t.repeat_len, t.copies, t.mat, t.mis, t.ins);
                const float qq = rr_ratio(t);
                if (best_ratio < qq) { bestr = t; best_ratio = qq; }
                loop_join();
            }
            if (!ok) { dp_too_large(c); rr_clear(bestr); }
            store(g, bestr, ok);
            if (lane_id() == 0) {
                c.wc[CNT_DP_CALLS] += 2ull; c.wc[CNT_DP_CELLS] += 2ull * (unsigned long long)rows * (unsigned long long)U;
                c.wc[CNT_DP_ROWS] += 2ull * (unsigned long long)rows; c.wc[CNT_TB_STEPS] += (unsigned long long)tb;
            }
        }
    }
    wc_time(c.wc, CYC_DP_TB, t_b);
}
DEVINL void dp_two_params_batch(K2Ctx &c, int qs, int qe, int n, unsigned ents)
{
    const int *pmeta = (const int *)(c.sc + c.y.pool_meta);
    Dp4 q; q.n = n;
    int ent[4], kk[4];
#pragma unroll
    for (int g = 0; g < 4; g++) {
        ent[g] = (int)((ents >> (5 * g)) & 31u);
        const int e = g < n ? ent[g] : ent[0];
        q.U[g] = g < n ? uni(pmeta[4 * e]) : 1;
        kk[g] = uni(pmeta[4 * e + 1]);
        q.unit[g] = slot_unit(c, K2_NSLOT_FIXED + e);
        q.off[g] = 0;
    }
    dp_two_params_q4(c, qs, qe, q, kk, [&](int g, const RR &bestr, bool ok) {
        if (ok) memo_store(c, q.unit[g], q.U[g], bestr);
        pool_store(c, ent[g], bestr);
    });
}
DEVINL unsigned unit_key16(const uint8_t *ub, int U)
{
    const int lane = lane_id();
    const int b = lane < U ? (int)ub[lane] : 0;
    const unsigned lo = (unsigned)__ballot((b & 1) != 0), hi = (unsigned)__ballot((b & 2) != 0);
    return (lo & 0xffffu) | (hi << 16);
}

DEVINL int search_walks(K2Ctx &c, int qs, int qe, int k, int &max_freq_out, int &n_ent, int (&e_of)[2])
{
    const int lane = lane_id();
    int max_freq = tab_build(c, k, qs, qe);
    max_freq_out = max_freq;
    int found = 0;
    e_of[0] = -1; e_of[1] = -1;
    int *pmeta = (int *)(c.sc + c.y.pool_meta);
    if (MTRC_MIN_NUM_FREQ_UNIT < max_freq) {
        int ns = tab_seeds(c, k, qs, qe, max_freq);
        int found_bwd = 0;
        for (int turn = 0; turn < 2; turn++) {
            const int dir = 1 - turn;
            if (turn == 1 && !found_bwd) break;
            for (int s = 0; s < ns; s++) {
                int seed = uni(c.seeds[s]);
                int period = walk(c, dir == 1, qs, qe, k, seed, K2_NSLOT_FIXED + n_ent);
                found = period > 0 ? 1 : 0;
                if (!found && s + MTRC_SCREEN_MIN_SEEDS < ns) {
                    s = screen_seeds(c, dir == 1, qs, qe, k, s + 1, ns) - 1;
                }
                if (found) {
                    if (period < MTRC_MIN_PERIOD) {
                        wc_add(c.wc, CNT_MEMO_HITS, 1);
                        wc_add(c.wc, CNT_MEMO_CELLS, 2ll * (long long)(qe - qs + 1) * (long long)period);
                        break;
                    }
                    if (lane == 0) { pmeta[4 * n_ent] = period; pmeta[4 * n_ent + 1] = k; pmeta[4 * n_ent + 2] = dir; }
                    e_of[dir] = n_ent;
                    n_ent++;
                    break;
                }
                loop_join();
            }
            if (dir == 1) found_bwd = found;
            loop_join();
        }
        found = found_bwd;
    }
    return found;
}


#define POL_OUT_OFF 512
static_assert(MTRC_MAX_PERIOD <= POL_OUT_OFF, "a staged unit and its polished form share the look-ahead's staging bytes");
DEVINL int pol_base(const lds_u8 *st, int j) { return uni((int)st[j]) & 3; }
DEVINL int pol_score(const lds_u8 *st, int j) { return (uni((int)st[j]) >> 2) & 3; }
DEVINL void wave_sync_lds()
{
    asm volatile("s_waitcnt lgkmcnt(0)" ::: "memory");
    __builtin_amdgcn_wave_barrier();
}
struct PolMask {
    long long v;
    DEVINL unsigned long long word(int q) const { return (unsigned long long)lane_val64(v, q); }
};
struct PolOps {
    const K2Ctx *c; const lds_u8 *st; lds_u8 *out; int k, period;
    DEVINL int base(int j) const { return pol_base(st, j); }
    DEVINL int score(int j) const { return pol_score(st, j); }
    DEVINL int get(int node) const { return uni(tab_get(*c, node)); }
    DEVINL void get4(int a0, int a1, int a2, int a3, int &f0, int &f1, int &f2, int &f3) const
    {
#ifdef MTR_POLISH_WALK_ALL
        f0 = get(a0); f1 = get(a1); f2 = get(a2); f3 = get(a3);
#else
        const int lane = lane_id();
        const int key = lane == 0 ? a0 : lane == 1 ? a1 : lane == 2 ? a2 : a3;
        int v = 0;
        if (lane < 4) v = tab_get(*c, key);
        f0 = lane_val(v, 0); f1 = lane_val(v, 1); f2 = lane_val(v, 2); f3 = lane_val(v, 3);
#endif
    }
    DEVINL int cyc(int j) const
    {
        const int lane = lane_id();
        const bool on = lane < 2 * k;
        int pos = j + (k - 1 - (lane >> 1)); if (pos >= period) pos -= period;
        const int b = on ? (int)st[pos] : 0;
        return (int)(unsigned)__ballot(on && ((b >> (lane & 1)) & 1) != 0);
    }
    DEVINL void emit(int jr, int b) const { if (lane_id() == 0) out[jr] = (unsigned char)b; }
    DEVINL void copy(int jr, int j, int n) const
    {
#pragma unroll 1
        for (int t = j - n + 1 + lane_id(); t <= j; t += 64) out[jr - j + t] = (unsigned char)(st[t] & 3);
    }
    DEVINL void undefined() const { wc_add(c->wc, CNT_UNDEFINED, 1); }
    DEVINL void join() const { loop_join(); }
};
DEVINL bool polish_staged(K2Ctx &c, const RR &r, const lds_u8 *st, lds_u8 *out, int &jr, unsigned long long t_stage)
{
    const int lane = lane_id();
    const int k = r.kmer, period = r.period;
    PolMask m; m.v = 0ll;
    unsigned long long any = 0ull;
#pragma unroll 1
    for (int q = 0; q * 64 < period; q++) {
        const int t = q * 64 + lane;
        const unsigned long long w = __ballot(t < period && pp_flagged([&](int p) { return ((int)st[p] >> 2) & 3; }, k, t));
        if (lane == q) m.v = (long long)w;
        any |= w;
    }
    const bool none = any == 0ull;
    wc_time_pol(c.wc, CNT_SPARE45, t_stage);
    if (none) return false;
    const unsigned long long t_tab = clk();
    (void)tab_build(c, k, r.rep_start, r.rep_end);
    wc_time_pol(c.wc, CNT_SPARE46, t_tab);
    const unsigned long long t_walk = clk();
    PolOps ops{&c, st, out, k, period};
    bool altered = false;
#ifdef MTR_POLISH_WALK_ALL
    const bool ok = pp_walk_all(ops, k, period, jr, altered);
#else
    const bool ok = pp_walk_plan(ops, m, k, period, jr, altered);
#endif
    wave_sync_lds();
    wc_time_pol(c.wc, CNT_SPARE47, t_walk);
    return ok && altered;
}

DEVINL void polish(K2Ctx &c, RR &r, int slot = 1)
{
    const int lane = lane_id();
    const int k = r.kmer, period = r.period;
    if (period <= k) return;
    uint8_t *ub = slot_unit(c, slot); const int *score = slot_score(c, slot);
    lds_u8 *st = (lds_u8 *)c.stage, *out = st + POL_OUT_OFF;
    const unsigned long long t_stage = clk();
#pragma unroll 1
    for (int t = lane; t < period; t += 64) st[t] = pp_stage_byte((int)ub[t], score[t]);
    wave_sync_lds();
    int jr = 0;
    if (!polish_staged(c, r, st, out, jr, t_stage)) return;
    const int np = (MTRC_MAX_PERIOD - 1) - jr;
#pragma unroll 1
    for (int t = lane; t < np; t += 64) ub[t] = out[t + jr + 1];
    wave_sync_mem();
    r.period = np;
}

DEVINL int min_missing(int period, double err, int coverage)
{
    int a = period > 200 ? 0 : period > 150 ? 1 : period > 100 ? 2 : period > 75 ? 3 : period > 50 ? 4 :
            period > 30 ? 5 : period > 20 ? 6 : period > 10 ? 7 : period > 5 ? 8 : 9;
    int b = err > 0.25 ? 0 : err > 0.225 ? 1 : err > 0.2 ? 2 : err > 0.175 ? 3 : err > 0.15 ? 4 :
            err > 0.125 ? 5 : err > 0.1 ? 6 : err > 0.075 ? 7 : err > 0.05 ? 8 : 9;
    int cc = coverage <= 1 ? 0 : coverage >= 20 ? 19 : coverage - 1;
    return (int)d_min_missing[(a * 10 + b) * 20 + cc] - '0';
}

DEVINL int revise_threshold(const RR &t)
{
    if (t.period <= 0) return 0x7fffffff;
    const int coverage = t.repeat_len / t.period;
    if (!(5 <= coverage && coverage <= 20)) return 0x7fffffff;
    return min_missing(t.period, (double)(t.mis + t.ins + t.del) / (double)t.repeat_len, coverage);
}
DEVINL void revise_tally(K2Ctx &c, RR &t, int U, lds_int *lv, const int *cons, const int *miss, int slot, bool &unchanged)
{
    const int lane = lane_id();
    uint8_t *ub = slot_unit(c, slot);
    const unsigned long long t0 = clk();
    const int thr = revise_threshold(t);
    int *rev = (int *)(c.sc + c.y.pol_rev);
    int n = 0;
    for (int base = 1; base <= U; base += 64) {
        int j = base + lane;
        int e0 = -1, e1 = -1;
        if (j <= U) {
            int mv = -1, mb = -1;
            for (int q = 0; q < 5; q++) { int v = lv ? lv[j * 5 + q] : cons[j * 5 + q]; if (mv < v) { mv = v; mb = q; } }
            if (mb < 4) e0 = mb;
            mv = -1; int mm = -1;
            for (int q = 0; q < 4; q++) { int v = lv ? lv[(U + 1) * 5 + j * 4 + q] : miss[j * 4 + q]; if (mv < v) { mv = v; mm = q; } }
            if (thr != 0x7fffffff && thr <= mv && 0 <= mm && mm <= 3) e1 = mm;
        }
        int cntl = (e0 >= 0 ? 1 : 0) + (e1 >= 0 ? 1 : 0);
        int pre = cntl;
        for (int d = 1; d < 64; d <<= 1) { int o2 = __shfl_up(pre, d, 64); if (lane >= d) pre += o2; }
        int pos = n + pre - cntl;
        if (e0 >= 0) { rev[pos] = e0; pos++; }
        if (e1 >= 0) rev[pos] = e1;
        n += lane_val(pre, 63);
    }
    wave_sync_mem();
    bool diff = false;
    for (int tt = lane; tt < n && tt < K2_SLOT_UNIT; tt += 64) { diff = diff || (ub[tt] != (uint8_t)rev[tt]); ub[tt] = (uint8_t)rev[tt]; }
    unchanged = (n == U) && (__ballot(diff) == 0ull);
    wc_add(c.wc, CNT_SPARE44, 1);
    if (unchanged) wc_add(c.wc, CNT_SPARE43, 1);
    wave_sync_mem();
    t.period = n;
    wc_time(c.wc, CYC_REVISE_VOTE, t0);
}
DEVINL bool revise_sub(K2Ctx &c, RR &t, int G, int MM, int D, DpRes &dp, bool &unchanged, int slot = 3)
{
    const int U = t.period, rs = t.rep_start, re = t.rep_end;
    t.G = G; t.MM = MM; t.D = D;
    int *cons = (int *)(c.sc + c.y.cons), *miss = (int *)(c.sc + c.y.miss);
    uint8_t *ub = slot_unit(c, slot);
    DpRes o;
    lds_int *lv = ((U + 1) * 9 <= K2_TAB_CAP) ? c.lds_keys : (lds_int *)nullptr;
    bool okdp = dp_wrap(c.pk, rs, re - rs + 1, ub, U, G, MM, D, c.sc + c.y.codes, c.y.cells, 1, cons, miss, lv, o, c.wc, c.a->dp16_max_rows);
    if (!okdp) { dp_too_large(c); return false; }
    revise_tally(c, t, U, lv, cons, miss, slot, unchanged);
    dp = o;
    trace_ev(c, 5, rs, re, U, G, MM, D, t.period, trace_on(c, 5) && t.period > 0 && t.period < K2_SLOT_UNIT ? unit_hash(ub, t.period) : 0, 0, 0, 0, 0, 0, 0);
    return true;
}

DEVINL bool round_lookup(K2Ctx &c, int p, RR &t, int &valid)
{
    const int lane = lane_id();
// ... 212 lines not shown
    if (!((st.found_mask >> ki) & 1u)) rr_clear(cur);
    else if ((long long)cur.period * (long long)(qe - qs + 1) > mtr_dev_wrap_dp_size) rr_clear(cur);
    else if (cur.period == 0) rr_clear(cur);
    else {
        const int coverage = cur.repeat_len / cur.period;
        return 5 <= coverage && coverage <= 20 && 5 < cur.period;
    }
    return false;
}
DEVINL bool k2_better(const K2Args &a, float best_ratio, const RR &cur)
{
    const float q = rr_ratio(cur);
    return best_ratio < q && a.min_match_ratio <= q && MTRC_MIN_NUM_FREQ_UNIT < cur.copies && MTRC_MIN_PERIOD <= cur.period;
}
DEVINL bool k2_qualifies(const RR &best) { return best.repeat_len > 0 && best.rep_start + MTRC_MIN_PERIOD * MTRC_MIN_NUM_FREQ_UNIT < best.rep_end; }

DEVINL bool k2_range_select(K2Ctx &c, int qs, int qe, const RangeP1 &st, RR &best)
{
    const K2Args &a = *c.a;
    rr_clear(best);
    float best_ratio = -1.0f;
    c.rmemo_n = 0;
    for (int k = st.min_k; k <= st.max_k; k++) {
        if (!((st.run_mask >> (k - st.min_k)) & 1u)) continue;
        RR cur; int k_slot;
        if (k2_select_k(c, qs, qe, st, k, cur, k_slot, true)) revise(c, cur);
        if (k2_better(a, best_ratio, cur)) { best_ratio = rr_ratio(cur); best = cur; slot_copy(c, 0, 1); }
        loop_join();
    }
    return k2_qualifies(best);
}

DEVINL bool k2_range(K2Ctx &c, int qs, int qe, int w, RR &best)
{
    RangeP1 st;
    k2_range_walks(c, qs, qe, w, st);
    k2_range_dps(c, qs, qe, st);
    return k2_range_select(c, qs, qe, st, best);
}

DEVINL void prune_ranges(const int32_t *rs, int32_t *re, int t, int nr, int rep_start, int rep_end)
{
    const int lane = lane_id();
    for (int base = t + 1; base < nr; base += 64) {
        int u = base + lane;
        if (u < nr) {
            int s2 = rs[u], e2 = re[u];
            if (s2 >= rep_start && s2 < rep_end && e2 >= 0 && e2 < rep_end) re[u] = -1;
        }
    }
    wave_sync_mem();
}

DEVINL void k2_read(K2Ctx &c)
{
    const K2Args &a = *c.a;
    const int lane = lane_id();
    const int rd = c.rd;
    const int nr = uni(a.r_count[rd]);
    const int64_t off = uni64(a.r_off[rd]);
    const int32_t *rs = a.r_start + off; int32_t *re = a.r_end + off; const int32_t *rw = a.r_w + off;
    int nrec = 0;
    c.memo_n = 0; c.memo_qs = c.memo_qe = -1; c.memo_U = 0;
    for (int t = 0; t < nr; t++) {
        const int qs = uni(rs[t]), qe = uni(re[t]), w = uni(rw[t]);
        if (qe < 0) continue;
        RR best;
        const bool rec = k2_range(c, qs, qe, w, best);
        wc_add(c.wc, CNT_RANGES_EXEC, 1);
        if (rec) {
            emit_record(c, best, nrec); nrec++;
            trace_ev(c, 6, best.rep_start, best.rep_end, best.repeat_len, best.period, best.copies, best.mat, best.mis, best.ins, best.del, best.kmer, best.G, best.MM, best.D, trace_on(c, 6) ? unit_hash(slot_unit(c, 0), best.period) : 0);
            prune_ranges(rs, re, t, nr, best.rep_start, best.rep_end);
        }
        loop_join();
    }
    if (lane == 0) a.rec_count[rd] = nrec;
    wc_add(c.wc, CNT_RECORDS, nrec);
}

template <bool MANHATTAN>
__global__ __launch_bounds__(64, MTR_WAVES_PER_SIMD) void mtr_k_reads(K1Args a1, K2Args a)
{
    __shared__ __attribute__((aligned(16))) int s_arena[MTR_ARENA_INTS];
    __shared__ unsigned long long s_cnt[CNT_N];
    static_assert(MTR_ARENA_INTS == K2_TAB_CAP + MTRC_MAX_SEEDS + 4 + 4 * 64, "arena layout");
    int *s_keys = s_arena, *s_seeds = s_arena + K2_TAB_CAP, *s_stage = s_seeds + MTRC_MAX_SEEDS + 4;
    if (lane_id() < CNT_N) s_cnt[lane_id()] = 0ull;
    K2Ctx c;
    c.a = &a;
    c.wc = s_cnt;
    c.sc = a.scratch + (size_t)blockIdx.x * a.scratch_per_wave;
    c.y = k2_layout(a.Lmax);
    c.lds_keys = (lds_int *)s_keys; c.seeds = (lds_int *)s_seeds; c.stage = (lds_int *)s_stage;
    c.ties = (int *)(c.sc + c.y.ties); c.fresh = c.ties + MTRC_MAX_TIEBREAKS;
    for (;;) {
        const int t = next_work_item(a.work_counter);
        if (t >= a.b.n_reads) break;
        c.rd = uni(a.b.order[t]);
        c.L = uni(a.b.lens[c.rd]);
        c.pk = a.b.packed + uni64(a.b.woff[c.rd]);
        const unsigned long long t_read = clk();
#ifdef MTR_PROFILE
        const unsigned long long rt_read = __builtin_amdgcn_s_memrealtime();
#endif
        k1_read<MANHATTAN>(a1, c.rd, c.sc, (lds_u8 *)s_arena, MTR_ARENA_INTS * 4, s_cnt);
        wave_sync_mem();
        k2_read(c);
        wc_time(s_cnt, CYC_TOTAL, t_read);
#ifdef MTR_PROFILE
        wc_add(s_cnt, CNT_RESERVED15, (long long)(__builtin_amdgcn_s_memrealtime() - rt_read));
#endif
        trace_ev(c, 7, (int)(s_cnt[CYC_TOTAL] >> 10), (int)(s_cnt[CYC_DP_FWD] >> 10), (int)(s_cnt[CYC_DP_TB] >> 10),
                 (int)(s_cnt[CYC_DP_FWD_REV] >> 10), (int)(s_cnt[CYC_DP_TB_REV] >> 10), (int)(s_cnt[CYC_TAB_BUILD] >> 10),
                 (int)(s_cnt[CYC_WALK] >> 10), (int)s_cnt[CNT_DP_CALLS], (int)(s_cnt[CNT_DP_CELLS] >> 10), (int)(s_cnt[CNT_LOOKUPS] >> 10),
                 (int)s_cnt[CNT_TABLES], (int)s_cnt[CNT_RANGES_EXEC], (int)s_cnt[CNT_TB_STEPS], c.L);
        if (a.trace_cap > 0) wc_flush(s_cnt, a.counters);
        loop_join();
    }
    wc_flush(s_cnt, a.counters);
}

__global__ __launch_bounds__(64, MTR_WAVES_PER_SIMD) void mtr_k_units(K2Args a)
{
    __shared__ __attribute__((aligned(16))) int s_arena[MTR_ARENA_INTS];
    __shared__ unsigned long long s_cnt[CNT_N];
    int *s_keys = s_arena, *s_seeds = s_arena + K2_TAB_CAP, *s_stage = s_seeds + MTRC_MAX_SEEDS + 4;
    if (lane_id() < CNT_N) s_cnt[lane_id()] = 0ull;
    K2Ctx c;
    c.a = &a;
    c.wc = s_cnt;
    c.sc = a.scratch + (size_t)blockIdx.x * a.scratch_per_wave;
    c.y = k2_layout(a.Lmax);
    c.lds_keys = (lds_int *)s_keys; c.seeds = (lds_int *)s_seeds; c.stage = (lds_int *)s_stage;
    c.ties = (int *)(c.sc + c.y.ties); c.fresh = c.ties + MTRC_MAX_TIEBREAKS;
    for (;;) {
        const int t = next_work_item(a.work_counter);
        if (t >= a.b.n_reads) break;
        c.rd = uni(a.b.order[t]);
        c.L = uni(a.b.lens[c.rd]);
        c.pk = a.b.packed + uni64(a.b.woff[c.rd]);
        const unsigned long long t_read = clk();
        k2_read(c);
        wc_time(s_cnt, CYC_TOTAL, t_read);
        loop_join();
    }
    wc_flush(s_cnt, a.counters);
}

struct SplitArgs {
    const int64_t *item_off;
    DevRecord *cand;
    int32_t *cand_flag;
};

template <typename L, typename F>
DEVINL long long replay_ranges(int32_t *re, int nr, L &&flag_of, F &&on_record)
{
    const int lane = lane_id();
    long long executed = 0;
    for (int base = 0; base < nr; base += 64) {
        const int t = base + lane;
        const bool valid = t < nr;
        int e_l = valid ? re[t] : -1;
        const int f_l = valid ? flag_of(t) : 0;
        int pos = 0;
        while (pos < 64) {
            const unsigned long long behind = ~0ull << pos;
            const unsigned long long alive = __ballot(valid && e_l >= 0) & behind;
            const unsigned long long marked = __ballot(valid && e_l >= 0 && f_l != 0) & behind;
            if (marked == 0ull) { executed += __popcll(alive); break; }
            const int j = first_lane(marked);
            executed += __popcll(alive & ((1ull << j) - 1ull)) + 1;
            if (!on_record(base + j, lane_val(f_l, j))) return executed;
            if (valid) e_l = re[t];
            pos = j + 1;
            loop_join();
        }
        loop_join();
    }
    return executed;
}

__global__ __launch_bounds__(64) void mtr_k_replay(K2Args a, SplitArgs s)
{
    const int lane = lane_id();
    if (uni(*(volatile int32_t *)a.status) == DEV_ERR_STAGED_OVERFLOW) return;
    for (int rd = blockIdx.x; rd < a.b.n_reads; rd += gridDim.x) {
        int hv = 0; long long ho = 0;
        if (lane == 0) { hv = a.r_count[rd]; ho = a.r_off[rd]; } else if (lane == 1) ho = s.item_off[rd];
        const int nr = lane_val(hv, 0);
        const int64_t off = lane_val64(ho, 0), first = lane_val64(ho, 1);
        const int32_t *rs = a.r_start + off; int32_t *re = a.r_end + off;
        int nrec = 0;
        bool sent_back = false;
        const int32_t *flags = s.cand_flag + first;
        const long long executed = replay_ranges(re, nr, [&](int t) -> int { return flags[t]; }, [&](int t, int flag) -> bool {
            if (flag < 0) {
                sent_back = true;
                return false;
            }
            const DevRecord *src = s.cand + (flag - 1);
            if (nrec < a.max_rec_per_read) {
                const int64_t base = a.rec_base ? uni64(a.rec_base[rd]) : (int64_t)rd * (int64_t)a.max_rec_per_read;
                const uint4 *sp = (const uint4 *)src;
                uint4 *dp = (uint4 *)(a.records + base + nrec);
                for (int q = lane; q < (int)(sizeof(DevRecord) / 16); q += 64) dp[q] = sp[q];
            }
            nrec++;
            const int rep_start = uni(src->f[0]), rep_end = uni(src->f[1]);
// ... 63 lines not shown
```

### mtr_amd/csrc/k3_staged.hip.inc

```
#pragma once
#include "k2_units.hip.inc"
#include "dp_quad.hip.inc"

#define ST_QCLASSES 8
#define ST_QROWBINS 2048
#define ST_QSUB 8
#define ST_NBINS (ST_QCLASSES * ST_QROWBINS * ST_QSUB)
#define ST_QUMAX 128
#define ST_OUMAX 32
#define ST_OCLS0 (ST_QCLASSES - 2)

struct StItemHdr {
    int32_t n_slots; uint32_t run_mask, found_mask; int32_t min_k, max_k;
    int32_t rd, t, qs, qe, w, item, stride;
    long long pad0, pad1;
};
struct StEnt { int32_t period, k, dir, dpi; };
struct StK { int32_t state, slot; int32_t rr[14]; long long rev_off; };
struct StRev { long long block; int32_t k, slot; int32_t rr[14]; long long leader; int32_t ri, pad[3]; };
#define ST_REV_BYTES ((long long)sizeof(StRev) + K2_SLOT_UNIT + 4ll * K2_SLOT_SCORE)
struct StDpItem { int32_t rd, qs, rows, U; long long unit_off, codes_off; int32_t best[6]; int32_t pad[2]; };
static_assert(sizeof(StItemHdr) == 64 && sizeof(StEnt) == 16 && sizeof(StDpItem) == 64 && sizeof(StK) == 72 && sizeof(StRev) == 96, "staged layouts");

struct StagedArgs {
// ... 170 lines not shown
            s.cand_flag[first + t] = p ? -1 : 0;
            if (p == 0) atomicAdd(&n_p0, 1);
        }
        __syncthreads();
        if (threadIdx.x == 0) p0_base = (int)atomicAdd(s.n_pass[0], (unsigned)n_p0);
        __syncthreads();
        if (threadIdx.x == 0) n_p0 = 0;
        __syncthreads();
        for (int t = threadIdx.x; t < nr; t += blockDim.x)
            if (s.item_pass[first + t] == 0) { const int q = atomicAdd(&n_p0, 1); s.pass_list[0][p0_base + q] = (int32_t)(first + t); }
        __syncthreads();
    }
}

__global__ __launch_bounds__(64) void mtr_k_pass_mark(K2Args a, StagedArgs s)
{
    const int lane = lane_id();
    if (st_staged_overflowed(a)) return;
    for (int rd = blockIdx.x; rd < s.n_reads; rd += gridDim.x) {
        int hv = 0; long long ho = 0;
        if (lane == 0) { hv = a.r_count[rd]; ho = a.r_off[rd]; } else if (lane == 1) ho = s.item_off[rd];
        const int nr = lane_val(hv, 0);
        const int64_t off = lane_val64(ho, 0), first = lane_val64(ho, 1);
        const int32_t *rs = a.r_start + off; int32_t *re = s.re2 + off;
        for (int t = lane; t < nr; t += 64) re[t] = a.r_end[off + t];
        wave_sync_mem();
        (void)replay_ranges(re, nr,
            [&](int t) -> int { const int flag = s.cand_flag[first + t]; return s.item_pass[first + t] == 0 && flag > 0 ? flag : 0; },
            [&](int t, int flag) -> bool {
                const DevRecord *src = s.cand + (flag - 1);
                prune_ranges(rs, re, t, nr, uni(src->f[0]), uni(src->f[1]));
                return true;
            });
        if (s.test_flags & 1) continue;
        int n_need = 0;
        for (int base = 0; base < nr; base += 64) {
            const int t = base + lane;
            n_need += __popcll(__ballot(t < nr && re[t] >= 0 && s.item_pass[first + t] != 0));
        }
        if (n_need == 0) continue;
        unsigned b0 = 0;
        if (lane == 0) b0 = atomicAdd(s.n_pass[1], (unsigned)n_need);
        b0 = (unsigned)uni((int)b0);
        for (int base = 0; base < nr; base += 64) {
            const int t = base + lane;
            const bool need = t < nr && re[t] >= 0 && s.item_pass[first + t] != 0;
            const unsigned long long m = __ballot(need);
            if (need) s.pass_list[1][b0 + (unsigned)mbcnt(m)] = (int32_t)(first + t);
            b0 += (unsigned)__popcll(m);
        }
    }
}

DEVINL int st_max_unit(int qs, int qe)
{
    int u = (qe - qs) / MTRC_MIN_NUM_FREQ_UNIT; if (u > MTRC_MAX_PERIOD) u = MTRC_MAX_PERIOD; if (u < 1) u = 1;
    return u;
}
DEVINL uint8_t *st_slot_unit(uint8_t *arena, long long base, const StItemHdr *h, int sid)
{
    return arena + base + (long long)sizeof(StItemHdr) + (long long)sizeof(StEnt) * h->n_slots + (long long)sid * h->stride;
}
DEVINL StK *st_ktab(uint8_t *arena, long long base, const StItemHdr *h)
{
    return (StK *)(arena + base + (long long)sizeof(StItemHdr) + (long long)sizeof(StEnt) * h->n_slots + (long long)h->n_slots * h->stride);
}
DEVINL void st_rr_store(int32_t *o, const RR &r)
{
    if (lane_id() == 0) {
        o[0] = r.rep_start; o[1] = r.rep_end; o[2] = r.repeat_len; o[3] = r.period; o[4] = r.copies; o[5] = r.mat; o[6] = r.mis;
        o[7] = r.ins; o[8] = r.del; o[9] = r.kmer; o[10] = r.G; o[11] = r.MM; o[12] = r.D; o[13] = 0;
    }
}
DEVINL void st_rr_load(const int32_t *o, RR &x)
{
    const int lane = lane_id();
    const int v = lane < 13 ? o[lane] : 0;
    x.rep_start = lane_val(v, 0); x.rep_end = lane_val(v, 1); x.repeat_len = lane_val(v, 2); x.period = lane_val(v, 3);
    x.copies = lane_val(v, 4); x.mat = lane_val(v, 5); x.mis = lane_val(v, 6); x.ins = lane_val(v, 7); x.del = lane_val(v, 8);
    x.kmer = lane_val(v, 9); x.G = lane_val(v, 10); x.MM = lane_val(v, 11); x.D = lane_val(v, 12);
}
DEVINL void st_park_entries(K2Ctx &c, const StagedArgs &s, long long base, const RangeP1 &st, int min_k, int stride, int n_slots, int maxU)
{
    const int lane = lane_id();
    const int *pmeta = (const int *)(c.sc + c.y.pool_meta);
    StEnt *en = (StEnt *)(s.arena + base + sizeof(StItemHdr));
    for (int e = 0; e < st.n_ent; e++) {
        const int U = uni(pmeta[4 * e]), k = uni(pmeta[4 * e + 1]), dir = uni(pmeta[4 * e + 2]);
        const int sid = 2 * (k - min_k) + dir;
        if (sid < 0 || sid >= n_slots || U > maxU) { set_status(c.a->status, DEV_ERR_INTERNAL); continue; }
        const uint8_t *ub = slot_unit(c, K2_NSLOT_FIXED + e); const int *us = slot_score(c, K2_NSLOT_FIXED + e);
        uint8_t *du = s.arena + base + (long long)sizeof(StItemHdr) + (long long)sizeof(StEnt) * n_slots + (long long)sid * stride;
        int *ds = (int *)(du + st_pad16(maxU));
        {
            int sv[8], bv[8];
#pragma unroll
            for (int q = 0; q < 8; q++) {
                const int t = q * 64 + lane, f = dir == 1 ? U - 1 - t : t;
                sv[q] = t < U ? us[f] : 0; bv[q] = t < U ? (int)ub[f] : 0;
            }
#pragma unroll
            for (int q = 0; q < 8; q++) { const int t = q * 64 + lane; if (t < U) { du[t] = (uint8_t)bv[q]; ds[t] = sv[q]; } }
        }
        if (lane == 0) { en[sid].period = U; en[sid].k = k; en[sid].dir = dir; en[sid].dpi = -1; }
        loop_join();
    }
    wave_sync_mem();
}

#define WS_PER_LANE 4
__global__ __launch_bounds__(64) void mtr_k_walk_screen(K2Args a, StagedArgs s)
{
    const int lane = lane_id();
    const int n_items = s.two_pass ? (int)uni((int)*s.n_pass[s.pass]) : uni(*s.n_items);
    const int32_t *src = s.two_pass ? s.pass_list[s.pass] : nullptr;
    int n_dead = 0, n_skipped = 0;
    for (long long base = (long long)blockIdx.x * (64 * WS_PER_LANE); base < (long long)n_items; base += (long long)gridDim.x * (64 * WS_PER_LANE)) {
        int it_l[WS_PER_LANE]; bool keep[WS_PER_LANE]; int n_keep = 0;
        int4 rec[WS_PER_LANE]; int L_l[WS_PER_LANE]; long long woff_l[WS_PER_LANE];
#pragma unroll
        for (int r = 0; r < WS_PER_LANE; r++) {
            const long long q = base + 64 * r + lane;
            it_l[r] = q < (long long)n_items ? (src ? src[q] : (int)q) : -1;
        }
#pragma unroll
        for (int r = 0; r < WS_PER_LANE; r++) rec[r] = it_l[r] >= 0 ? s.item_tab[it_l[r]] : make_int4(0, 0, 0, 0);
#pragma unroll
        for (int r = 0; r < WS_PER_LANE; r++) { L_l[r] = it_l[r] >= 0 ? a.b.lens[rec[r].x] : 0; woff_l[r] = it_l[r] >= 0 ? a.b.woff[rec[r].x] : 0; }
#pragma unroll
        for (int r = 0; r < WS_PER_LANE; r++) {
            const int qs = rec[r].y, qe = rec[r].z, w = rec[r].w;
            const bool have = it_l[r] >= 0;
            bool dead = false;
            if (have && ws_applies(qs, qe, w)) dead = ws_range_dead(a.b.packed + woff_l[r], L_l[r], qs, qe, w, nullptr);
            if (dead) s.cand_flag[it_l[r]] = 0;
            keep[r] = have && !dead;
            const unsigned long long dm = __ballot(dead), d100 = __ballot(dead && w >= 100);
            int mk_lo, mk_hi, mk0;
            k2_k_range(0, mk0, mk_lo); k2_k_range(100, mk0, mk_hi);
            n_dead += __popcll(dm);
            n_skipped += (__popcll(dm) - __popcll(d100)) * (mk_lo - mk0) + __popcll(d100) * (mk_hi - mk0);
            n_keep += __popcll(__ballot(keep[r]));
        }
        if (n_keep == 0) continue;
        unsigned got = 0;
        if (lane == 0) got = atomicAdd(s.n_walk, (unsigned)n_keep);
        got = (unsigned)uni((int)got);
        if ((long long)got + (long long)n_keep > (long long)s.walk_cap) { set_status(a.status, DEV_ERR_STAGED_OVERFLOW); break; }
#pragma unroll
        for (int r = 0; r < WS_PER_LANE; r++) {
            const unsigned long long m = __ballot(keep[r]);
            if (keep[r]) s.walk_list[got + (unsigned)mbcnt(m)] = it_l[r];
            got += (unsigned)__popcll(m);
        }
    }
    if (n_dead > 0 && lane < 3) {
        const int which = lane == 0 ? CNT_SPARE54 : lane == 1 ? CNT_TABLES : CNT_TABLES_SKIPPED;
        atomicAdd(&a.counters[which], (unsigned long long)(lane == 2 ? n_skipped : n_dead));
    }
}

__global__ __launch_bounds__(64, MTR_LAT_WAVES_PER_SIMD) void mtr_k_walks(K2Args a, StagedArgs s)
{
    __shared__ __attribute__((aligned(16))) int s_arena[MTR_ARENA_INTS];
    __shared__ unsigned long long s_cnt[CNT_N];
    int *s_keys = s_arena, *s_seeds = s_arena + K2_TAB_CAP, *s_stage = s_seeds + MTRC_MAX_SEEDS + 4;
    const int lane = lane_id();
    if (lane < CNT_N) s_cnt[lane] = 0ull;
    K2Ctx c;
    c.a = &a; c.wc = s_cnt; c.staged_walks = true;
    c.sc = a.scratch + (size_t)blockIdx.x * a.scratch_per_wave;
    c.y = k2_layout(a.Lmax, a.cells_cap);
    c.lds_keys = (lds_int *)s_keys; c.seeds = (lds_int *)s_seeds; c.stage = (lds_int *)s_stage;
    c.ties = (int *)(c.sc + c.y.ties); c.fresh = c.ties + MTRC_MAX_TIEBREAKS;
    if (s.walk_screen && st_staged_overflowed(a)) return;
    const int32_t *src = s.walk_screen ? s.walk_list : s.two_pass ? s.pass_list[s.pass] : nullptr;
    const int n_items = s.walk_screen ? (int)uni((int)*s.n_walk) : s.two_pass ? (int)uni((int)*s.n_pass[s.pass]) : uni(*s.n_items);
    Wq wq; wq_init(wq, (unsigned)n_items);
    constexpr int WB = 4;
    for (;;) {
        const long long qi0 = wq_next_batch(ST_WQ(s, 0), (unsigned)n_items, wq, (unsigned)WB);
        if (qi0 < 0) break;
        const long long myq = qi0 + (long long)lane * (long long)wq.nq;
        const bool have = lane < WB && myq < (long long)n_items;
        int it_l = 0, L_l = 0; int4 rec_l = make_int4(0, 0, 0, 0); long long ioff_l = 0, woff_l = 0;
        if (have) {
            it_l = src ? src[myq] : (int)myq;
            rec_l = s.item_tab[it_l];
            ioff_l = s.item_off[rec_l.x]; L_l = a.b.lens[rec_l.x]; woff_l = a.b.woff[rec_l.x];
        }
        const int n_have = __popcll(__ballot(have));
#pragma unroll 1
        for (int b = 0; b < n_have; b++) {
        const int it = lane_val(it_l, b);
        wc_add(c.wc, CNT_SPARE54, 1);
        c.rd = lane_val(rec_l.x, b);
        const int qs = lane_val(rec_l.y, b), qe = lane_val(rec_l.z, b), w = lane_val(rec_l.w, b);
        const int t = it - (int)lane_val64(ioff_l, b);
        c.L = lane_val(L_l, b);
        c.pk = a.b.packed + lane_val64(woff_l, b);
        c.memo_n = 0; c.memo_qs = c.memo_qe = -1; c.memo_U = 0;
        int min_k, max_k;
        k2_k_range(w, min_k, max_k);
        const int k_last = min_k + s.k_first - 1 < max_k ? min_k + s.k_first - 1 : max_k;
        RangeP1 st;
        int bound = 0x3fffffff;
#ifdef MTR_PROFILE_WALK_WIDTH
        const unsigned long long t_w = clk();
#endif
        k2_range_walks(c, qs, qe, w, st, min_k, k_last, 0x3fffffff, &bound);
#ifdef MTR_PROFILE_WALK_WIDTH
        { const int wd_ = qe - qs + 1; wc_time(c.wc, wd_ < 32 ? CNT_SPARE43 : wd_ < 64 ? CNT_SPARE44 : wd_ < 128 ? CNT_SPARE45 : wd_ < 256 ? CNT_SPARE46 : CNT_SPARE55, t_w); }
#endif
        if (lane == 0) s.cand_flag[it] = 0;
        unsigned alive = 0u;
        for (int k = k_last + 1; k <= max_k; k++) {
            const int lim = qe < c.L - k + 1 ? qe : c.L - k + 1;
            if (bound + (qe - lim + 1) > MTRC_MIN_NUM_FREQ_UNIT) alive |= 1u << (k - min_k);
            else { wc_add(c.wc, CNT_TABLES_SKIPPED, 1); trace_ev(c, 2, qs, qe, k, 0, 0, -1, -1, -1, -1, -1, -1, -1, -1, -1); }
        }
        if (st.n_ent == 0 && alive == 0u && trace_on(c, 2))
            for (int k = min_k; k <= k_last; k++) if ((st.run_mask >> (k - min_k)) & 1u)
                trace_ev(c, 2, qs, qe, k, (int)((st.found_mask >> (k - min_k)) & 1u), 0, -1, -1, -1, -1, -1, -1, -1, -1, -1);
        if (st.n_ent > 0 || alive != 0u) {
            const int n_slots = 2 * (max_k - min_k + 1), maxU = st_max_unit(qs, qe);
            const int stride = (int)(st_pad16(maxU) + st_pad16(4ll * maxU));
            const long long bytes = (long long)sizeof(StItemHdr) + (long long)sizeof(StEnt) * n_slots + (long long)n_slots * stride + (long long)sizeof(StK) * (n_slots / 2);
            const int n_alive = __builtin_popcount(alive);
            const long long base = st_reserve_bytes(s, bytes);
            const long long slot = st_reserve(s, ST_SL_KC, s.kc_cap, 1u);
            const long long cbase = n_alive ? st_reserve(s, st_sl_cont(st_cost_class(qe - qs + 1)), s.cont_cap, (unsigned)n_alive) : 0;
            if (base < 0 || slot < 0 || cbase < 0) set_status(a.status, DEV_ERR_STAGED_OVERFLOW);
            else {
                StItemHdr *h = (StItemHdr *)(s.arena + base);
                StEnt *en = (StEnt *)(h + 1);
                if (lane < n_slots) { en[lane].period = 0; en[lane].k = min_k + (lane >> 1); en[lane].dir = lane & 1; en[lane].dpi = -1; }
                if (lane == 0) {
                    h->n_slots = n_slots; h->run_mask = st.run_mask; h->found_mask = st.found_mask; h->min_k = min_k; h->max_k = max_k;
                    h->rd = c.rd; h->t = t; h->qs = qs; h->qe = qe; h->w = w; h->item = it; h->stride = stride; h->pad0 = 0; h->pad1 = 0;
                    s.kc_items[slot] = base;
                    size_t q = (size_t)st_cost_class(qe - qs + 1) * (size_t)s.cont_cap + cbase;
                    for (int k = k_last + 1; k <= max_k; k++)
                        if ((alive >> (k - min_k)) & 1u) s.cont[q++] = make_int4((int)(unsigned)(base & 0xffffffffll), (int)(base >> 32), k, bound);
                }
                wave_sync_mem();
                st_park_entries(c, s, base, st, min_k, stride, n_slots, maxU);
            }
        }
        loop_join();
        }
        loop_join();
    }
    wc_flush(s_cnt, a.counters);
}

__global__ __launch_bounds__(64, MTR_WAVES_PER_SIMD) void mtr_k_walks_k(K2Args a, StagedArgs s)
{
    __shared__ __attribute__((aligned(16))) int s_arena[MTR_ARENA_INTS];
    __shared__ unsigned long long s_cnt[CNT_N];
    int *s_keys = s_arena, *s_seeds = s_arena + K2_TAB_CAP, *s_stage = s_seeds + MTRC_MAX_SEEDS + 4;
    const int lane = lane_id();
    if (lane < CNT_N) s_cnt[lane] = 0ull;
    if (st_staged_overflowed(a)) return;
    K2Ctx c;
    c.a = &a; c.wc = s_cnt; c.staged_walks = true;
#ifdef MTR_PROFILE_WALK_FMT
    c.prof_kernel = 1;
#endif
    c.sc = a.scratch + (size_t)blockIdx.x * a.scratch_per_wave;
    c.y = k2_layout(a.Lmax, a.cells_cap);
    c.lds_keys = (lds_int *)s_keys; c.seeds = (lds_int *)s_seeds; c.stage = (lds_int *)s_stage;
    c.ties = (int *)(c.sc + c.y.ties); c.fresh = c.ties + MTRC_MAX_TIEBREAKS;
    for (int cls = ST_NCLS - 1; cls >= 0; cls--) {
    WqS wq;
    if (wqs_init(wq, s, st_sl_cont(cls), s.cont_cap) == 0) continue;
    for (;;) {
        const long long wi = wqs_next(s, ST_Q_WK + cls, s.cont_cap, wq);
        if (wi < 0) break;
        int4 rec = make_int4(0, 0, 0, 0);
        if (lane == 0) rec = s.cont[(size_t)cls * (size_t)s.cont_cap + wi];
        const long long base = (long long)(((unsigned long long)(unsigned)uni(rec.y) << 32) | (unsigned)uni(rec.x));
        const int k = uni(rec.z), bound = uni(rec.w);
        StItemHdr *h = (StItemHdr *)(s.arena + base);
        c.rd = uni(h->rd);
        const int qs = uni(h->qs), qe = uni(h->qe), w = uni(h->w), min_k = uni(h->min_k), n_slots = uni(h->n_slots), stride = uni(h->stride);
        c.L = uni(a.b.lens[c.rd]);
        c.pk = a.b.packed + uni64(a.b.woff[c.rd]);
        c.memo_n = 0; c.memo_qs = c.memo_qe = -1; c.memo_U = 0;
        RangeP1 st;
#ifdef MTR_PROFILE_WALK_WIDTH
        const unsigned long long t_w = clk();
#endif
        k2_range_walks(c, qs, qe, w, st, k, k, bound);
#ifdef MTR_PROFILE_WALK_WIDTH
        { const int wd_ = qe - qs + 1; wc_time(c.wc, wd_ < 32 ? CNT_SPARE43 : wd_ < 64 ? CNT_SPARE44 : wd_ < 128 ? CNT_SPARE45 : wd_ < 256 ? CNT_SPARE46 : CNT_SPARE55, t_w); }
#endif
        if (lane == 0) { if (st.run_mask) atomicOr(&h->run_mask, st.run_mask); if (st.found_mask) atomicOr(&h->found_mask, st.found_mask); }
        if (st.n_ent > 0) st_park_entries(c, s, base, st, min_k, stride, n_slots, st_max_unit(qs, qe));
        loop_join();
    }
    loop_join();
    }
    wc_flush(s_cnt, a.counters);
}

DEVINL unsigned st_rotl(unsigned x, int r) { return (x << r) | (x >> (32 - r)); }
__global__ __launch_bounds__(64) void mtr_k_gather(K2Args a, StagedArgs s)
{
    const int lane = lane_id();
    if (st_staged_overflowed(a)) return;
    WqS wq; (void)wqs_init(wq, s, ST_SL_KC, s.kc_cap);
    for (;;) {
        const long long wi = wqs_next(s, 8, s.kc_cap, wq);
        if (wi < 0) break;
        const long long base = uni64(s.kc_items[wi]);
        StItemHdr *h = (StItemHdr *)(s.arena + base);
        StEnt *en = (StEnt *)(h + 1);
        int hv = 0;
        if (lane < 12) hv = ((const int32_t *)h)[lane];
        const int n_slots = lane_val(hv, 0), min_k = lane_val(hv, 3), rd = lane_val(hv, 5), qs = lane_val(hv, 7), qe = lane_val(hv, 8), stride = lane_val(hv, 11);
        const unsigned found_mask = (unsigned)lane_val(hv, 2);
        const int rows = qe - qs + 1;
        const int ns = n_slots < 32 ? n_slots : 32;
        int Ue = 0, ke = min_k;
        if (lane < ns) { Ue = en[lane].period; ke = en[lane].k; }
        uint8_t *slot0 = s.arena + base + (long long)sizeof(StItemHdr) + (long long)sizeof(StEnt) * n_slots;
        const bool cand_l = lane < ns && Ue >= MTRC_MIN_PERIOD && ((found_mask >> (ke - min_k)) & 1u);
        const unsigned candm = (unsigned)__ballot(cand_l);
        if (candm == 0u) { loop_join(); continue; }
        unsigned h1 = 0u, h2 = 0u;
        if (cand_l) {
            const uint32_t *uw = (const uint32_t *)(slot0 + (long long)lane * stride);
            const int nw = (Ue + 3) >> 2;
            const uint32_t last_mask = (Ue & 3) ? ((1u << (8 * (Ue & 3))) - 1u) : 0xffffffffu;
            int q = 0;
            for (; q + 4 <= nw; q += 4) {
                uint32_t w0 = uw[q], w1 = uw[q + 1], w2 = uw[q + 2], w3 = uw[q + 3];
                if (q + 4 == nw) w3 &= last_mask;
                h1 = st_rotl((h1 ^ w0) * 0x9E3779B1u, 13); h2 = (h2 + w0) * 0x85EBCA77u; h2 ^= h2 >> 15;
                h1 = st_rotl((h1 ^ w1) * 0x9E3779B1u, 13); h2 = (h2 + w1) * 0x85EBCA77u; h2 ^= h2 >> 15;
                h1 = st_rotl((h1 ^ w2) * 0x9E3779B1u, 13); h2 = (h2 + w2) * 0x85EBCA77u; h2 ^= h2 >> 15;
                h1 = st_rotl((h1 ^ w3) * 0x9E3779B1u, 13); h2 = (h2 + w3) * 0x85EBCA77u; h2 ^= h2 >> 15;
            }
// ... 400 lines not shown
    if (lane < CNT_N) s_cnt[lane] = 0ull;
    if (st_staged_overflowed(a)) return;
    K2Ctx c;
    c.a = &a; c.wc = s_cnt;
    c.sc = a.scratch + (size_t)blockIdx.x * a.scratch_per_wave;
    c.y = k2_layout(a.Lmax, a.cells_cap);
    c.lds_keys = nullptr; c.seeds = nullptr; c.stage = nullptr; c.ties = nullptr; c.fresh = nullptr;
    st_dp2_waves_body(c, a, s);
    const int oct0 = uni(s.quad_cls[ST_OCLS0]);
    const unsigned nq4 = (unsigned)(oct0 >> 2), nq = nq4 + (unsigned)((uni(s.quad_cls[ST_QCLASSES]) - oct0) >> 3);
    if (nq == 0u) { wc_flush(s_cnt, a.counters); return; }
    Wq wq; wq_init(wq, nq);
    const unsigned q_stride = s.pass_shuffle ? st_scatter_stride(nq) : 1u;
    for (;;) {
        const int wi = wq_next(ST_WQ(s, ST_Q_QUAD), nq, wq);
        if (wi < 0) break;
        const unsigned pi = st_scatter_index((unsigned)wi, nq, q_stride);
        const bool oct = pi >= nq4;
        const int slot0 = oct ? oct0 + (int)((pi - nq4) << 3) : (int)pi << 2;
        bool fits = true;
        if (oct) fits = st_oct_run(c, a, s, slot0);
        else if (uni(s.sorted[slot0]) >= 0) {
        DpQuad q; q.n = 0;
        int items[4], kk[4];
        int maxrows = 0;
#pragma unroll
        for (int g = 0; g < 4; g++) {
            const int di = uni(s.sorted[slot0 + g]);
            items[g] = di;
            const StDpItem *d = s.dp + (di >= 0 ? di : uni(s.sorted[slot0]));
            const int rd = uni(d->rd);
            q.pk[g] = a.b.packed + uni64(a.b.woff[rd]);
            q.wlim[g] = (long long)a.packed_words - uni64(a.b.woff[rd]);
            q.base[g] = uni(d->qs); q.rows[g] = di >= 0 ? uni(d->rows) : 0; q.U[g] = uni(d->U);
            q.unit[g] = s.arena + uni64(d->unit_off);
            kk[g] = uni(d->pad[0]);
            if (di >= 0) { q.n = g + 1; maxrows = q.rows[g] > maxrows ? q.rows[g] : maxrows; }
        }
        const int C = DPQ_COLS(q.U[0]) < 3 ? 3 : DPQ_COLS(q.U[0]);
        fits = DPQ_BLOCK_BYTES(C, maxrows) <= c.y.cells;
        if (fits) switch (C) {
        case 3: st_quad_run<3>(c, a, s, items, q, kk, maxrows); break;
        case 4: st_quad_run<4>(c, a, s, items, q, kk, maxrows); break;
        case 5: st_quad_run<5>(c, a, s, items, q, kk, maxrows); break;
        case 6: st_quad_run<6>(c, a, s, items, q, kk, maxrows); break;
        case 7: st_quad_run<7>(c, a, s, items, q, kk, maxrows); break;
        default: st_quad_run<8>(c, a, s, items, q, kk, maxrows); break;
        }
        }
        if (!fits) {
#pragma unroll 1
            for (int g = 0; g < (oct ? 8 : 4); g++) {
                const int di = uni(s.sorted[slot0 + g]);
                if (di >= 0) {
                    const StDpItem *d = s.dp + di;
                    c.rd = uni(d->rd); c.L = uni(a.b.lens[c.rd]); c.pk = a.b.packed + uni64(a.b.woff[c.rd]);
                    const int qs = uni(d->qs), rows = uni(d->rows);
                    RR r; rr_clear(r); r.period = uni(d->U); r.kmer = uni(d->pad[0]);
                    dp_two_params_unit(c, qs, qs + rows - 1, r, s.arena + uni64(d->unit_off));
                    int *o = s.dp_res + (size_t)di * 16;
                    if (lane == 0) {
                        o[0] = r.rep_start; o[1] = r.rep_end; o[2] = r.repeat_len; o[3] = r.period; o[4] = r.copies; o[5] = r.mat; o[6] = r.mis;
                        o[7] = r.ins; o[8] = r.del; o[9] = r.kmer; o[10] = r.G; o[11] = r.MM; o[12] = r.D;
                    }
                }
                loop_join();
            }
        }
        loop_join();
    }
    wc_flush(s_cnt, a.counters);
}

DEVINL void st_list_rev_block(const K2Args &a, const StagedArgs &s, long long base)
{
    const long long slot = st_reserve(s, ST_SL_RB, s.kc_cap, 1u);
    if (slot < 0) set_status(a.status, DEV_ERR_STAGED_OVERFLOW);
    else if (lane_id() == 0) s.rb_items[slot] = base;
}
__global__ __launch_bounds__(64, MTR_WAVES_PER_SIMD) void mtr_k_select(K2Args a, StagedArgs s)
{
    __shared__ __attribute__((aligned(16))) int s_arena[MTR_ARENA_INTS];
    __shared__ unsigned long long s_cnt[CNT_N];
    int *s_keys = s_arena, *s_seeds = s_arena + K2_TAB_CAP, *s_stage = s_seeds + MTRC_MAX_SEEDS + 4;
    const int lane = lane_id();
    if (lane < CNT_N) s_cnt[lane] = 0ull;
    if (st_staged_overflowed(a)) return;
    K2Ctx c;
    c.a = &a; c.wc = s_cnt;
    c.sc = a.scratch + (size_t)blockIdx.x * a.scratch_per_wave;
    c.y = k2_layout(a.Lmax, a.cells_cap);
    c.lds_keys = (lds_int *)s_keys; c.seeds = (lds_int *)s_seeds; c.stage = (lds_int *)s_stage;
    c.ties = (int *)(c.sc + c.y.ties); c.fresh = c.ties + MTRC_MAX_TIEBREAKS;
    const bool quads = s.quad_min > 0;
    WqS wq; (void)wqs_init(wq, s, ST_SL_KC, s.kc_cap);
    for (;;) {
        const long long wi = wqs_next(s, 5, s.kc_cap, wq);
        if (wi < 0) break;
        const long long base = uni64(s.kc_items[wi]);
        const StItemHdr *h = (const StItemHdr *)(s.arena + base);
        const StEnt *en = (const StEnt *)(h + 1);
        int hv = 0;
        if (lane < 12) hv = ((const int32_t *)h)[lane];
        const int n_slots = lane_val(hv, 0), min_k = lane_val(hv, 3), rd = lane_val(hv, 5), qs = lane_val(hv, 7), qe = lane_val(hv, 8), item = lane_val(hv, 10);
        const unsigned run_mask = (unsigned)lane_val(hv, 1), found_mask = (unsigned)lane_val(hv, 2);
        const int rows = qe - qs + 1, nk = n_slots >> 1, stride = lane_val(hv, 11);
        uint8_t *slot0 = s.arena + base + (long long)sizeof(StItemHdr) + (long long)sizeof(StEnt) * n_slots;
        int Ue = 0, ke = min_k, dpi = -1;
        if (lane < n_slots && lane < 64) { Ue = en[lane].period; ke = en[lane].k; dpi = en[lane].dpi; }
        const bool has = Ue > 0;
        const bool fnd = has && ((found_mask >> (ke - min_k)) & 1u);
        if (n_slots > 64 || (n_slots & 1) || __ballot(fnd && dpi < 0) != 0ull) {
            set_status(a.status, DEV_ERR_STAGED_OVERFLOW);
            loop_join();
            continue;
        }
        c.rd = rd;
        int r0 = -1, r1 = -1, r2 = -1, r3 = -1, r4 = -1, r5 = -1, r6 = -1, r7 = -1, r8 = -1, r9 = -1, r10 = -1, r11 = -1, r12 = -1;
        if (fnd) {
            const int4 *o = (const int4 *)(s.dp_res + (size_t)(dpi & ~ST_DPI_DUP) * 16);
            const int4 v0 = o[0], v1 = o[1], v2 = o[2]; const int v3 = ((const int *)o)[12];
            r0 = v0.x; r1 = v0.y; r2 = v0.z; r3 = v0.w; r4 = v1.x; r5 = v1.y; r6 = v1.z; r7 = v1.w; r8 = v2.x; r9 = v2.y; r10 = v2.z; r11 = v2.w; r12 = v3;
            if (r3 != -1) { r9 = ke; r3 = Ue; }
        }
        {
            const bool memo = has && (!fnd || (dpi & ST_DPI_DUP));
            const unsigned long long mm = __ballot(memo);
            if (mm != 0ull) { wc_add(c.wc, CNT_MEMO_HITS, __popcll(mm)); wc_add(c.wc, CNT_MEMO_CELLS, wave_sum_i64(memo ? 2ll * (long long)rows * (long long)Ue : 0ll)); }
        }
        const int ki = lane, k = min_k + ki;
        const int s0 = (2 * ki) & 63, s1 = (2 * ki + 1) & 63;
        const bool in_k = ki < nk;
        const bool has0 = __shfl((int)has, s0, 64) != 0 && in_k, has1 = __shfl((int)has, s1, 64) != 0 && in_k;
        int c0 = -1, c1 = -1, c2 = -1, c3 = -1, c4 = -1, c5 = -1, c6 = -1, c7 = -1, c8 = -1, c9 = -1, c10 = -1, c11 = -1, c12 = -1, k_slot = -1;
        float k_ratio = -1.0f;
#define ST_SEL_DIR(HAS, SRC, E)                                                                                                                        \
        {                                                                                                                                              \
            const int t0 = __shfl(r0, SRC, 64), t1 = __shfl(r1, SRC, 64), t2 = __shfl(r2, SRC, 64), t3 = __shfl(r3, SRC, 64), t4 = __shfl(r4, SRC, 64),     \
                      t5 = __shfl(r5, SRC, 64), t6 = __shfl(r6, SRC, 64), t7 = __shfl(r7, SRC, 64), t8 = __shfl(r8, SRC, 64), t9 = __shfl(r9, SRC, 64),     \
                      t10 = __shfl(r10, SRC, 64), t11 = __shfl(r11, SRC, 64), t12 = __shfl(r12, SRC, 64);                                                  \
            const float q = (float)t5 / (float)(t5 + t6 + t7 + t8);                                                                                        \
            if ((HAS) && k_ratio < q && a.min_match_ratio <= q && MTRC_MIN_NUM_FREQ_UNIT < t4 && MTRC_MIN_PERIOD <= t3 && t3 < MTRC_MAX_PERIOD) {          \
                k_ratio = q; k_slot = (E);                                                                                                                 \
                c0 = t0; c1 = t1; c2 = t2; c3 = t3; c4 = t4; c5 = t5; c6 = t6; c7 = t7; c8 = t8; c9 = t9; c10 = t10; c11 = t11; c12 = t12;                 \
            }                                                                                                                                              \
        }
        ST_SEL_DIR(has0, s0, 2 * ki)
        ST_SEL_DIR(has1, s1, 2 * ki + 1)
#undef ST_SEL_DIR
        const bool run = in_k && ((run_mask >> ki) & 1u);
        if (trace_on(c, 2))
            for (int q = 0; q < nk; q++) if ((run_mask >> q) & 1u)
                trace_ev(c, 2, qs, qe, min_k + q, (int)((found_mask >> q) & 1u), 0, lane_val(c3, q), lane_val(c0, q), lane_val(c1, q), lane_val(c2, q), lane_val(c4, q), lane_val(c5, q), lane_val(c6, q), lane_val(c7, q), lane_val(c8, q));
        bool rev = false;
        {
            bool clear = false;
            if (!in_k || !((found_mask >> ki) & 1u)) clear = true;
            else if ((long long)c3 * (long long)rows > mtr_dev_wrap_dp_size) clear = true;
            else if (c3 == 0) clear = true;
            else { const int coverage = c2 / c3; rev = run && 5 <= coverage && coverage <= 20 && 5 < c3; }
            if (clear) { c0 = c1 = c2 = c3 = c4 = c5 = c6 = c7 = c8 = c9 = c10 = c11 = c12 = -1; }
        }
        const unsigned long long revm = __ballot(rev);
        long long ro = -1;
        if (revm != 0ull) {
            const unsigned n_rev = (unsigned)__popcll(revm);
            const long long ro0 = st_reserve_bytes(s, (long long)n_rev * ST_REV_BYTES);
            long long ri = -1;
            if (quads) { const long long r0l = st_reserve(s, ST_SL_REV, s.rev_cap, n_rev); ri = r0l < 0 ? -1 : r0l + (long long)mbcnt(revm); }
            else {
                for (unsigned long long m = revm; m != 0ull; m &= m - 1ull) {
                    const int l = first_lane(m);
                    const int rcls = st_cost_class(lane_val(c1, l) - lane_val(c0, l) + 1);
                    unsigned got = 0; if (lane == 0) got = atomicAdd(s.n_rev + rcls * ST_CLS_STRIDE, 1u); got = (unsigned)uni((int)got);
                    if (lane == l) ri = got < (unsigned)s.rev_cap ? (long long)got : -1;
                    loop_join();
                }
            }
            const bool bad = rev && (ro0 < 0 || ri < 0 || (quads && ri >= (long long)s.dp_cap));
            if (__ballot(bad) != 0ull) set_status(a.status, DEV_ERR_STAGED_OVERFLOW);
            else if (rev) {
                ro = ro0 + (long long)mbcnt(revm) * ST_REV_BYTES;
                StRev *rv = (StRev *)(s.arena + ro);
                const int rcls = quads ? 0 : st_cost_class(c1 - c0 + 1);
                rv->block = base; rv->k = k; rv->slot = k_slot; rv->leader = -1; rv->ri = (int32_t)ri;
                rv->rr[0] = c0; rv->rr[1] = c1; rv->rr[2] = c2; rv->rr[3] = c3; rv->rr[4] = c4; rv->rr[5] = c5; rv->rr[6] = c6; rv->rr[7] = c7; rv->rr[8] = c8;
                rv->rr[9] = c9; rv->rr[10] = c10; rv->rr[11] = c11; rv->rr[12] = c12; rv->rr[13] = 0;
                s.rev_items[(size_t)rcls * (size_t)s.rev_cap + (size_t)ri] = ro;
                if (quads) s.dp_bin[ri] = -1;
            }
        }
        StK *kt = (StK *)(slot0 + (long long)n_slots * stride);
        if (in_k) {
            StK *x = kt + ki;
            if (!run) { x->state = 0; x->slot = -1; x->rev_off = -1; }
            else {
                x->state = (rev && ro >= 0) ? 2 : 1; x->slot = k_slot; x->rev_off = ro;
                x->rr[0] = c0; x->rr[1] = c1; x->rr[2] = c2; x->rr[3] = c3; x->rr[4] = c4; x->rr[5] = c5; x->rr[6] = c6; x->rr[7] = c7; x->rr[8] = c8;
                x->rr[9] = c9; x->rr[10] = c10; x->rr[11] = c11; x->rr[12] = c12; x->rr[13] = 0;
            }
        }
        if (__ballot(rev && ro >= 0) != 0ull) { wave_sync_mem(); st_list_rev_block(a, s, base); loop_join(); continue; }
        {
            RR best; rr_clear(best);
            float best_ratio = -1.0f;
            int best_e = -1;
            for (int q = 0; q < nk; q++) {
                if (!((run_mask >> q) & 1u)) continue;
                RR cur;
                cur.rep_start = lane_val(c0, q); cur.rep_end = lane_val(c1, q); cur.repeat_len = lane_val(c2, q); cur.period = lane_val(c3, q); cur.copies = lane_val(c4, q);
                cur.mat = lane_val(c5, q); cur.mis = lane_val(c6, q); cur.ins = lane_val(c7, q); cur.del = lane_val(c8, q); cur.kmer = lane_val(c9, q);
                cur.G = lane_val(c10, q); cur.MM = lane_val(c11, q); cur.D = lane_val(c12, q);
                if (k2_better(a, best_ratio, cur)) { best_ratio = rr_ratio(cur); best = cur; best_e = lane_val(k_slot, q); }
            }
            if (k2_qualifies(best) && best_e >= 0) {
                unsigned ci = 0;
                if (lane == 0) ci = atomicAdd(s.n_cand, 1u);
                ci = (unsigned)uni((int)ci);
                if (ci >= (unsigned)s.cand_cap) set_status(a.status, DEV_ERR_STAGED_OVERFLOW);
                else {
                    const uint8_t *bu = slot0 + (long long)best_e * stride;
                    emit_record_from(best, bu, (const int *)(bu + st_pad16(st_max_unit(qs, qe))), s.cand + ci);
                    if (lane == 0) s.cand_flag[item] = (int32_t)ci + 1;
                }
            }
        }
        wave_sync_mem();
        loop_join();
    }
    wc_flush(s_cnt, a.counters);
}

__global__ __launch_bounds__(64, MTR_WAVES_PER_SIMD) void mtr_k_revise(K2Args a, StagedArgs s)
{
    __shared__ __attribute__((aligned(16))) int s_arena[MTR_ARENA_INTS];
    __shared__ unsigned long long s_cnt[CNT_N];
    int *s_keys = s_arena, *s_seeds = s_arena + K2_TAB_CAP, *s_stage = s_seeds + MTRC_MAX_SEEDS + 4;
    const int lane = lane_id();
    if (lane < CNT_N) s_cnt[lane] = 0ull;
    if (st_staged_overflowed(a)) return;
    K2Ctx c;
    c.a = &a; c.wc = s_cnt;
    c.sc = a.scratch + (size_t)blockIdx.x * a.scratch_per_wave;
    c.y = k2_layout(a.Lmax, a.cells_cap);
    c.lds_keys = (lds_int *)s_keys; c.seeds = (lds_int *)s_seeds; c.stage = (lds_int *)s_stage;
    c.ties = (int *)(c.sc + c.y.ties); c.fresh = c.ties + MTRC_MAX_TIEBREAKS;
    for (int cls = ST_NCLS - 1; cls >= 0; cls--) {
    unsigned n_rev = s.n_rev[cls * ST_CLS_STRIDE]; if (n_rev > (unsigned)s.rev_cap) n_rev = (unsigned)s.rev_cap;
    n_rev = (unsigned)uni((int)n_rev);
    if (n_rev == 0u) continue;
    Wq wq; wq_init(wq, n_rev);
    for (;;) {
        const int wi = wq_next(ST_WQ(s, ST_Q_REV + cls), n_rev, wq);
        if (wi < 0) break;
        const long long ro = uni64(s.rev_items[(size_t)cls * (size_t)s.rev_cap + wi]);
        StRev *rv = (StRev *)(s.arena + ro);
        const long long base = uni64(rv->block);
        const StItemHdr *h = (const StItemHdr *)(s.arena + base);
        const StEnt *en = (const StEnt *)(h + 1);
        c.rd = uni(h->rd);
        c.L = uni(a.b.lens[c.rd]);
        c.pk = a.b.packed + uni64(a.b.woff[c.rd]);
        c.memo_n = 0; c.memo_qs = c.memo_qe = -1; c.memo_U = 0; c.rmemo_n = 0;
        const int e = uni(rv->slot), qs = uni(h->qs), qe = uni(h->qe);
        RR cur; st_rr_load(rv->rr, cur);
        {
            const int U = uni(en[e].period), maxU = st_max_unit(qs, qe);
            uint8_t *ub = slot_unit(c, 1); int *us = slot_score(c, 1);
            const uint8_t *su = st_slot_unit(s.arena, base, h, e); const int *ss = (const int *)(su + st_pad16(maxU));
            slot_load_candidate(ub, us, su, ss, U);
            wave_sync_mem();
        }
        revise(c, cur);
        st_rr_store(rv->rr, cur);
        {
            const uint32_t *su = (const uint32_t *)slot_unit(c, 1); uint32_t *du = (uint32_t *)(s.arena + ro + sizeof(StRev));
            const int *ss = slot_score(c, 1); int *ds = (int *)(s.arena + ro + sizeof(StRev) + K2_SLOT_UNIT);
            slot_copy_raw((uint8_t *)du, ds, (const uint8_t *)su, ss);
        }
        wave_sync_mem();
        loop_join();
    }
    loop_join();
    }
    wc_flush(s_cnt, a.counters);
}

DEVINL void st_member_ctx(K2Ctx &c, const K2Args &a, int rd) { c.rd = rd; c.L = uni(a.b.lens[rd]); c.pk = a.b.packed + uni64(a.b.woff[rd]); }
__global__ __launch_bounds__(64, MTR_LAT_WAVES_PER_SIMD) void mtr_k_polish(K2Args a, StagedArgs s)
{
    __shared__ __attribute__((aligned(16))) int s_arena[MTR_ARENA_INTS];
    __shared__ unsigned long long s_cnt[CNT_N];
    int *s_keys = s_arena, *s_seeds = s_arena + K2_TAB_CAP, *s_stage = s_seeds + MTRC_MAX_SEEDS + 4;
    const int lane = lane_id();
    if (lane < CNT_N) s_cnt[lane] = 0ull;
    if (st_staged_overflowed(a)) return;
    K2Ctx c;
    c.a = &a; c.wc = s_cnt;
    c.sc = a.scratch + (size_t)blockIdx.x * a.scratch_per_wave;
    c.y = k2_layout(a.Lmax, a.cells_cap);
    c.lds_keys = (lds_int *)s_keys; c.seeds = (lds_int *)s_seeds; c.stage = (lds_int *)s_stage;
    c.ties = (int *)(c.sc + c.y.ties); c.fresh = c.ties + MTRC_MAX_TIEBREAKS;
    c.memo_n = 0; c.memo_qs = c.memo_qe = -1; c.memo_U = 0; c.rmemo_n = 0;
    WqS wq; (void)wqs_init(wq, s, ST_SL_REV, s.rev_cap);
    for (;;) {
        const unsigned long long t_pull = clk();
        const long long wi = wqs_next(s, ST_Q_POLISH, s.rev_cap, wq);
        if (wi < 0) break;
        const long long ro = uni64(s.rev_items[wi]);
        StRev *rv = (StRev *)(s.arena + ro);
        const long long base = uni64(rv->block);
        const StItemHdr *h = (const StItemHdr *)(s.arena + base);
        const StEnt *en = (const StEnt *)(h + 1);
        st_member_ctx(c, a, uni(h->rd));
        const int e = uni(rv->slot), qs = uni(h->qs), qe = uni(h->qe);
        RR cur; st_rr_load(rv->rr, cur);
        wc_time_pol(c.wc, CNT_SPARE43, t_pull);
        const unsigned long long t_in = clk();
        const int U = uni(en[e].period), maxU = st_max_unit(qs, qe);
        uint8_t *du = s.arena + ro + sizeof(StRev); int *ds = (int *)(s.arena + ro + sizeof(StRev) + K2_SLOT_UNIT);
        lds_u8 *st = (lds_u8 *)c.stage, *out = st + POL_OUT_OFF;
        {
            const uint8_t *su = st_slot_unit(s.arena, base, h, e); const int *ss = (const int *)(su + st_pad16(maxU));
            int sv[K2_SLOT_SCORE / 64]; int bv[K2_SLOT_SCORE / 64];
#pragma unroll
            for (int q = 0; q < K2_SLOT_SCORE / 64; q++) { const int t = q * 64 + lane; sv[q] = t < U ? ss[t] : -1; bv[q] = t < U ? (int)su[t] : 0; }
#pragma unroll
            for (int q = 0; q < K2_SLOT_SCORE / 64; q++) { const int t = q * 64 + lane; ds[t] = sv[q]; if (t < POL_OUT_OFF) st[t] = pp_stage_byte(bv[q], sv[q]); }
        }
        wave_sync_lds();
        wc_time_pol(c.wc, CNT_SPARE44, t_in);
        const int in_period = cur.period;
        const unsigned long long t0 = clk();
        int jr = 0;
        const bool changed = cur.period > cur.kmer && polish_staged(c, cur, st, out, jr, t0);
        wc_time(c.wc, CYC_POLISH, t0);
        const unsigned long long t_out = clk();
        if (changed) {
            const int np = (MTRC_MAX_PERIOD - 1) - jr;
#pragma unroll 1
            for (int t = lane; t < np; t += 64) du[t] = out[t + jr + 1];
            cur.period = np;
            st_rr_store(rv->rr, cur);
        } else {
#pragma unroll 1
            for (int t = lane; t < U; t += 64) du[t] = (uint8_t)(st[t] & 3);
        }
        if (trace_on(c, 4)) {
            wave_sync_mem();
            trace_ev(c, 4, cur.rep_start, cur.rep_end, cur.kmer, in_period, cur.period, unit_hash(du, cur.period), 0, 0, 0, 0, 0, 0, 0, 0);
        }
        wave_sync_lds();
        wc_time_pol(c.wc, CNT_SPARE55, t_out);
        loop_join();
    }
    wc_flush(s_cnt, a.counters);
}

__global__ __launch_bounds__(64) void mtr_k_rev_share(K2Args a, StagedArgs s)
{
    __shared__ unsigned long long s_cnt[CNT_N];
    const int lane = lane_id();
    if (lane < CNT_N) s_cnt[lane] = 0ull;
    if (st_staged_overflowed(a)) return;
    WqS wq; (void)wqs_init(wq, s, ST_SL_RB, s.kc_cap);
    for (;;) {
        const long long wi = wqs_next(s, ST_Q_POLISH + 1, s.kc_cap, wq);
        if (wi < 0) break;
        const long long base = uni64(s.rb_items[wi]);
        const StItemHdr *h = (const StItemHdr *)(s.arena + base);
        int hv = 0;
        if (lane < 12) hv = ((const int32_t *)h)[lane];
        const int n_slots = lane_val(hv, 0), stride = lane_val(hv, 11);
        const int nk = n_slots / 2;
        const StK *kt = (const StK *)(s.arena + base + (long long)sizeof(StItemHdr) + (long long)sizeof(StEnt) * n_slots + (long long)n_slots * stride);
        long long ro_l = -1;
        if (lane < nk && lane < 32 && kt[lane].state == 2) ro_l = kt[lane].rev_off;
        const unsigned todo = (unsigned)__ballot(ro_l >= 0);
        int f0 = 0, f1 = 0, f2 = 0, f3 = 0, f4 = 0, f5 = 0, f6 = 0, f7 = 0, f8 = 0, f10 = 0, f11 = 0, f12 = 0, ri_l = 0;
        unsigned h1 = 0u, h2 = 0u;
        if (ro_l >= 0) {
            const StRev *rv = (const StRev *)(s.arena + ro_l);
            f0 = rv->rr[0]; f1 = rv->rr[1]; f2 = rv->rr[2]; f3 = rv->rr[3]; f4 = rv->rr[4]; f5 = rv->rr[5]; f6 = rv->rr[6]; f7 = rv->rr[7]; f8 = rv->rr[8];
            f10 = rv->rr[10]; f11 = rv->rr[11]; f12 = rv->rr[12]; ri_l = rv->ri;
            const uint32_t *uw = (const uint32_t *)(s.arena + ro_l + sizeof(StRev));
            const int U = f3 > 0 ? (f3 < K2_SLOT_UNIT ? f3 : K2_SLOT_UNIT) : 0;
            const int nw = (U + 3) >> 2;
            const uint32_t last_mask = (U & 3) ? ((1u << (8 * (U & 3))) - 1u) : 0xffffffffu;
            int q = 0;
            for (; q + 4 <= nw; q += 4) {
                uint32_t w0 = uw[q], w1 = uw[q + 1], w2 = uw[q + 2], w3 = uw[q + 3];
                if (q + 4 == nw) w3 &= last_mask;
                h1 = st_rotl((h1 ^ w0) * 0x9E3779B1u, 13); h2 = (h2 + w0) * 0x85EBCA77u; h2 ^= h2 >> 15;
                h1 = st_rotl((h1 ^ w1) * 0x9E3779B1u, 13); h2 = (h2 + w1) * 0x85EBCA77u; h2 ^= h2 >> 15;
                h1 = st_rotl((h1 ^ w2) * 0x9E3779B1u, 13); h2 = (h2 + w2) * 0x85EBCA77u; h2 ^= h2 >> 15;
                h1 = st_rotl((h1 ^ w3) * 0x9E3779B1u, 13); h2 = (h2 + w3) * 0x85EBCA77u; h2 ^= h2 >> 15;
            }
            for (; q < nw; q++) {
                uint32_t w0 = uw[q];
                if (q + 1 == nw) w0 &= last_mask;
                h1 = st_rotl((h1 ^ w0) * 0x9E3779B1u, 13); h2 = (h2 + w0) * 0x85EBCA77u; h2 ^= h2 >> 15;
            }
        }
        unsigned leaders = 0u;
        long long lead_l = -1;
        for (unsigned m = todo; m != 0u; m &= m - 1u) {
            const int ki = __builtin_ctz(m);
            const long long ro = lane_val64(ro_l, ki);
            const int U = lane_val(f3, ki);
            const bool same = lane_val(f0, ki) == f0 && lane_val(f1, ki) == f1 && lane_val(f2, ki) == f2 && U == f3 && lane_val(f4, ki) == f4 && lane_val(f5, ki) == f5 &&
                              lane_val(f6, ki) == f6 && lane_val(f7, ki) == f7 && lane_val(f8, ki) == f8 && lane_val(f10, ki) == f10 && lane_val(f11, ki) == f11 &&
                              lane_val(f12, ki) == f12 && (unsigned)lane_val((int)h1, ki) == h1 && (unsigned)lane_val((int)h2, ki) == h2;
            long long lead = -1;
            for (unsigned lm = (unsigned)__ballot(same) & leaders; lm != 0u && lead < 0; lm &= lm - 1u) {
                const long long lo = lane_val64(ro_l, __builtin_ctz(lm));
                const uint8_t *u1 = s.arena + ro + sizeof(StRev), *u2 = s.arena + lo + sizeof(StRev);
                bool diff = false;
                for (int q = lane; q < U; q += 64) diff = diff || (u1[q] != u2[q]);
                if (__ballot(diff) == 0ull) lead = lo;
                loop_join();
            }
            if (lead >= 0) { if (lane == ki) lead_l = lead; wc_add(s_cnt, CNT_REV_SHARED, 1); }
            else leaders |= 1u << ki;
            loop_join();
        }
        if (ro_l >= 0) {
            StRev *rv = (StRev *)(s.arena + ro_l);
            if (lead_l >= 0) { rv->leader = lead_l; s.dp_bin[ri_l] = -1; }
            else {
                const int rrows = f1 - f0 + 1;
                int rb = ST_QROWBINS - 1 - (rrows >> 3); if (rb < 0) rb = 0;
                const int cc = f3 > ST_QUMAX ? 8 : (f3 < 1 ? 1 : DPQ_COLS(f3));
                const int bin = ((8 - cc) * ST_QROWBINS + rb) * ST_QSUB + (int)(blockIdx.x & (ST_QSUB - 1));
                rv->leader = -1;
                s.dp_bin[ri_l] = bin; s.dp_rank[ri_l] = (int32_t)atomicAdd(s.bin_count + bin, 1u);
            }
        }
        loop_join();
    }
    wc_flush(s_cnt, a.counters);
}

enum { RS_EMPTY = 0, RS_VOTE = 1, RS_ALIGN = 2 };
struct StRevMember { int32_t state, round, id, quad, valid, unchanged; int32_t dp[8]; float base_ratio; int32_t pad; };
#define RQ_SLOTS 8
DEVINL void st_fwd1p_four(int C, const DpOct &o, uint8_t *cells, int maxrows, int (&best)[RQ_SLOTS][3])
{
    DpQuad q; q.n = o.n;
#pragma unroll
    for (int g = 0; g < 4; g++) {
        q.pk[g] = o.pk[g]; q.wlim[g] = o.wlim[g]; q.base[g] = o.base[g]; q.rows[g] = o.rows[g]; q.U[g] = o.U[g]; q.unit[g] = o.unit[g];
        q.G[g] = o.G[g]; q.MM[g] = o.MM[g]; q.D[g] = o.D[g];
    }
    int b4[4][3];
    switch (C) {
    case 1: dp_forward1p_g16<1, 16, DPQ_SCALE, true>(q, cells, maxrows, b4); break;
    case 2: dp_forward1p_g16<2, 16, DPQ_SCALE, true>(q, cells, maxrows, b4); break;
    case 3: dp_forward1p_g16<3, 16, DPQ_SCALE, true>(q, cells, maxrows, b4); break;
    case 4: dp_forward1p_g16<4, 16, DPQ_SCALE, true>(q, cells, maxrows, b4); break;
    case 5: dp_forward1p_g16<5, 16, DPQ_SCALE, true>(q, cells, maxrows, b4); break;
    case 6: dp_forward1p_g16<6, 16, DPQ_SCALE, true>(q, cells, maxrows, b4); break;
    case 7: dp_forward1p_g16<7, 16, DPQ_SCALE, true>(q, cells, maxrows, b4); break;
    default: dp_forward1p_g16<8, 16, DPQ_SCALE, true>(q, cells, maxrows, b4); break;
    }
#pragma unroll
    for (int g = 0; g < 4; g++) { best[g][0] = b4[g][0]; best[g][1] = b4[g][1]; best[g][2] = b4[g][2]; }
}
DEVINL void st_fwd1p_any(int C, const DpOct &q, uint8_t *cells, int maxrows, int (&best)[RQ_SLOTS][3])
{
    switch (C) {
    case 1: dp_forward1p_h8<1>(q, cells, maxrows, best); break;
    case 2: dp_forward1p_h8<2>(q, cells, maxrows, best); break;
    case 3: dp_forward1p_h8<3>(q, cells, maxrows, best); break;
    case 4: dp_forward1p_h8<4>(q, cells, maxrows, best); break;
    case 5: dp_forward1p_h8<5>(q, cells, maxrows, best); break;
    case 6: dp_forward1p_h8<6>(q, cells, maxrows, best); break;
    case 7: dp_forward1p_h8<7>(q, cells, maxrows, best); break;
    default: dp_forward1p_h8<8>(q, cells, maxrows, best); break;
    }
}
#define MTR_RQ_LDS_BYTES (RQ_SLOTS * 64 + CNT_N * 8)
static_assert(16 * MTR_ARENA_CORESIDENT_BYTES + 4 * MTR_LDS_ALLOC(MTR_RQ_LDS_BYTES) <= MTR_LDS_PER_CU, "four DP wavefronts beside sixteen arena wavefronts");
static_assert(16 * MTR_LDS_ALLOC(MTR_ARENA_INTS * 4 + CNT_N * 8) <= MTR_LDS_PER_CU, "sixteen wavefronts of an arena kernel per CU");
__global__ __launch_bounds__(64, MTR_WAVES_PER_SIMD) void mtr_k_revise_quads(K2Args a, StagedArgs s)
{
    typedef __attribute__((address_space(3))) StRevMember lds_StRevMember;
    __shared__ __attribute__((aligned(16))) StRevMember s_slots[RQ_SLOTS];
    __shared__ unsigned long long s_cnt[CNT_N];
    static_assert(sizeof(StRevMember) == 64 && sizeof(s_slots) + sizeof(s_cnt) == MTR_RQ_LDS_BYTES && MTR_RQ_LDS_BYTES <= 2048, "mtr_k_revise_quads: the LDS it uses, at most 2 KB");
    lds_StRevMember *s_mem = (lds_StRevMember *)s_slots;
    const int lane = lane_id();
    if (lane < CNT_N) s_cnt[lane] = 0ull;
    if (lane < RQ_SLOTS) { s_mem[lane].state = RS_EMPTY; s_mem[lane].round = 0; s_mem[lane].id = -1; }
    if (st_staged_overflowed(a)) return;
    K2Ctx c;
    c.a = &a; c.wc = s_cnt;
    c.sc = a.scratch + (size_t)blockIdx.x * a.scratch_per_wave;
    c.y = k2_layout(a.Lmax, a.cells_cap);
    c.lds_keys = nullptr; c.seeds = nullptr; c.stage = nullptr;
    c.ties = (int *)(c.sc + c.y.ties); c.fresh = c.ties + MTRC_MAX_TIEBREAKS;
    c.memo_n = 0; c.memo_qs = c.memo_qe = -1; c.memo_U = 0; c.rmemo_n = 0;
    const unsigned n_slots = (unsigned)uni(s.quad_cls[ST_QCLASSES]);
    if (n_slots == 0u) return;
    uint8_t *cells = c.sc + c.y.codes;
    int *cons = (int *)(c.sc + c.y.cons), *miss = (int *)(c.sc + c.y.miss);
    Wq wq; wq_init(wq, n_slots);
    bool list_empty = false;
    wave_sync_mem();
    const unsigned long long t_kernel = clk();
    for (;;) {
        const unsigned long long t_fill = clk();
        int n_active = 0;
#pragma unroll 1
        for (int g = 0; g < RQ_SLOTS; g++) {
            if (uni(s_mem[g].state) != RS_EMPTY) { n_active++; continue; }
            int id = -1;
            while (!list_empty && id < 0) {
                const int wi = wq_next(ST_WQ(s, ST_Q_QUAD + 1), n_slots, wq);
                if (wi < 0) list_empty = true; else id = uni(s.sorted[wi]);
                loop_join();
            }
            if (id < 0) continue;
            const long long ro = uni64(s.rev_items[id]);
            StRev *rv = (StRev *)(s.arena + ro);
            const long long base = uni64(rv->block);
            const StItemHdr *h = (const StItemHdr *)(s.arena + base);
            st_member_ctx(c, a, uni(h->rd));
            RR cur; st_rr_load(rv->rr, cur);
            const int S1 = K2_NSLOT_FIXED + 2 * g;
            {
                slot_copy_unit_raw(slot_unit(c, S1), s.arena + ro + sizeof(StRev));
                wave_sync_mem();
            }
            if (lane == 0) { s_mem[g].base_ratio = rr_ratio(cur); s_mem[g].state = RS_VOTE; s_mem[g].round = 0; s_mem[g].id = id; }
            pool_store(c, g, cur);
            wave_sync_mem();
            n_active++;
            loop_join();
        }
        wc_time_aux(c.wc, CNT_SPARE47, t_fill);
        if (n_active == 0) break;
        const unsigned long long t_prep = clk();
        DpOct q; q.n = RQ_SLOTS;
        int maxrows = 0, maxU = 0, n_quad = 0;
#pragma unroll 1
        for (int g = 0; g < RQ_SLOTS; g++) { q.pk[g] = a.b.packed; q.wlim[g] = 1; q.base[g] = 0; q.rows[g] = 0; q.U[g] = 0; q.unit[g] = c.sc; q.G[g] = 1; q.MM[g] = 1; q.D[g] = 1; }
#pragma unroll 1
        for (int g = 0; g < RQ_SLOTS; g++) {
            const int state = uni(s_mem[g].state);
            if (state == RS_EMPTY) continue;
            const int p = uni(s_mem[g].round);
            const int G = p == 0 ? 5 : 1, MM = 1, D = p == 0 ? 1 : 3;
            const long long ro = uni64(s.rev_items[uni(s_mem[g].id)]);
            const StItemHdr *h = (const StItemHdr *)(s.arena + uni64(((const StRev *)(s.arena + ro))->block));
            const int rd = uni(h->rd);
            st_member_ctx(c, a, rd);
            const int S3 = K2_NSLOT_FIXED + 2 * g + 1;
            RR t;
            if (state == RS_VOTE) { pool_load(c, g, t); slot_copy_unit(c, S3, K2_NSLOT_FIXED + 2 * g); }
            else pool_load(c, RQ_SLOTS + g, t);
            const int U = t.period, rows = t.rep_end - t.rep_start + 1;
            const bool fits = U >= 1 && U <= ST_QUMAX && rows >= 1 && rows <= a.dp16_max_rows && DPQ_FITS(rows, U, G, D) && (RQ_SLOTS / 4) * DPQP_BLOCK_BYTES(DPQ_COLS(U), rows) <= c.y.cells && dp_size_ok(U, rows);
            int quad = 0, valid = 0, unchanged = 0;
            if (fits) {
                const int k = n_quad;
                quad = k + 1;
// ... 254 lines not shown
```

Measured before the change: 305,800.

## Shrink unit-search LDS arena by spilling seeds and polish output to scratch

Reduces the per-wave LDS arena of the unit-search kernels by keeping only 16 seeds in LDS (the rest go to global scratch), packing look-ahead staged matches into one word and recomputing the digit, and nibble-packing polish staging with the polished output moved to global scratch. The aim is to fit more wavefronts per CU. The walks kernel's launch bound is also switched to the latency waves-per-SIMD setting, and wave_sum_i64 now uses ds_bpermute directly. In exchange, extra global memory traffic and recomputation in the hot paths, plus extra memory syncs.

```diff
diff --git a/mtr_amd/csrc/device_util.hip.inc b/mtr_amd/csrc/device_util.hip.inc
--- a/mtr_amd/csrc/device_util.hip.inc
+++ b/mtr_amd/csrc/device_util.hip.inc
@@ -9,6 +9,7 @@
 typedef __attribute__((address_space(3))) unsigned char lds_u8;
 
 DEVINL int lane_id() { return (int)(threadIdx.x & 63u); }
+DEVINL int lane_here() { int l = lane_id(); asm volatile("" : "+v"(l)); return l; }
 __device__ long long mtr_dev_wrap_dp_size = MTRC_WRAP_DP_SIZE;
 DEVINL bool dp_size_ok(int U, int rows) { return (size_t)(U + 1) * (size_t)rows + (size_t)U < (size_t)mtr_dev_wrap_dp_size; }
 DEVINL int uni(int v) { return __builtin_amdgcn_readfirstlane(v); }
@@ -51,7 +52,12 @@
 DEVINL int wave_max_i32_dpp(int v) { return lane_val((int)scan_max_u32((unsigned)(v + 1)), 63) - 1; }
 DEVINL long long wave_sum_i64(long long v)
 {
-    for (int d = 32; d > 0; d >>= 1) v += __shfl_xor(v, d, 64);
+    const int lane = lane_here();
+    for (int d = 32; d > 0; d >>= 1) {
+        const int at = (lane ^ d) << 2;
+        const unsigned lo = (unsigned)__builtin_amdgcn_ds_bpermute(at, (int)(unsigned)v), hi = (unsigned)__builtin_amdgcn_ds_bpermute(at, (int)(unsigned)((unsigned long long)v >> 32));
+        v += (long long)(((unsigned long long)hi << 32) | lo);
+    }
     return v;
 }
 
diff --git a/mtr_amd/csrc/dp_test.hip.inc b/mtr_amd/csrc/dp_test.hip.inc
--- a/mtr_amd/csrc/dp_test.hip.inc
+++ b/mtr_amd/csrc/dp_test.hip.inc
@@ -231,7 +231,7 @@
 {
     __shared__ __attribute__((aligned(16))) int s_arena[MTR_ARENA_INTS];
     __shared__ unsigned long long s_cnt[CNT_N];
-    int *s_keys = s_arena, *s_seeds = s_arena + K2_TAB_CAP, *s_stage = s_seeds + MTRC_MAX_SEEDS + 4;
+    int *s_keys = s_arena, *s_seeds = s_arena + K2_TAB_CAP, *s_stage = s_seeds + K2_SEEDS_LDS;
     const int lane = lane_id();
     if (lane < CNT_N) s_cnt[lane] = 0ull;
     K2Ctx c;
@@ -272,7 +272,7 @@
 {
     __shared__ __attribute__((aligned(16))) int s_arena[MTR_ARENA_INTS];
     __shared__ unsigned long long s_cnt[CNT_N];
-    int *s_keys = s_arena, *s_seeds = s_arena + K2_TAB_CAP, *s_stage = s_seeds + MTRC_MAX_SEEDS + 4;
+    int *s_keys = s_arena, *s_seeds = s_arena + K2_TAB_CAP, *s_stage = s_seeds + K2_SEEDS_LDS;
     const int lane = lane_id();
     if (lane < CNT_N) s_cnt[lane] = 0ull;
     K2Ctx c;
diff --git a/mtr_amd/csrc/k1_ranges.hip.inc b/mtr_amd/csrc/k1_ranges.hip.inc
--- a/mtr_amd/csrc/k1_ranges.hip.inc
+++ b/mtr_amd/csrc/k1_ranges.hip.inc
@@ -1169,11 +1169,17 @@
     wc_time(wc, CYC_K1_TOTAL, t_start);
 }
 
-#define MTR_ARENA_INTS (2048 + 104 + 256)
+#ifndef K2_SEEDS_LDS
+#define K2_SEEDS_LDS 16
+#endif
+#define K2_STAGE_INTS 64
+#define MTR_ARENA_INTS (2048 + K2_SEEDS_LDS + K2_STAGE_INTS)
+#define K1_ARENA_INTS (2048 + 104 + 256)
+static_assert(K1_ARENA_INTS >= MTR_ARENA_INTS, "the per-read kernel's arena holds the unit search's");
 
 __global__ __launch_bounds__(64, 4) void mtr_k1_part(K1Args a, int parts, const int32_t *item_read, const int32_t *item_pass, int n_items)
 {
-    __shared__ __attribute__((aligned(16))) int s_arena[MTR_ARENA_INTS];
+    __shared__ __attribute__((aligned(16))) int s_arena[K1_ARENA_INTS];
     __shared__ unsigned long long s_cnt[CNT_N];
     if (lane_id() < CNT_N) s_cnt[lane_id()] = 0ull;
     for (;;) {
@@ -1183,8 +1189,8 @@
         const int pv = item_pass ? __builtin_amdgcn_readfirstlane(item_pass[t]) : -1;
         const int ps = pv < 0 ? -1 : (pv & 255), seg = pv < 0 ? -1 : (pv >> 8) - 1;
         uint8_t *sc = a.scratch + (size_t)rd * a.scratch_per_wave;
-        if (a.manhattan) k1_read<true, true>(a, rd, sc, (lds_u8 *)s_arena, MTR_ARENA_INTS * 4, s_cnt, parts, ps, seg);
-        else k1_read<false, true>(a, rd, sc, (lds_u8 *)s_arena, MTR_ARENA_INTS * 4, s_cnt, parts, ps, seg);
+        if (a.manhattan) k1_read<true, true>(a, rd, sc, (lds_u8 *)s_arena, K1_ARENA_INTS * 4, s_cnt, parts, ps, seg);
+        else k1_read<false, true>(a, rd, sc, (lds_u8 *)s_arena, K1_ARENA_INTS * 4, s_cnt, parts, ps, seg);
         loop_join();
     }
     wc_flush(s_cnt, a.counters);
@@ -1293,7 +1299,7 @@
 
 __global__ __launch_bounds__(64, 4) void mtr_k1_ranges(K1Args a)
 {
-    __shared__ __attribute__((aligned(16))) int s_arena[MTR_ARENA_INTS];
+    __shared__ __attribute__((aligned(16))) int s_arena[K1_ARENA_INTS];
     __shared__ unsigned long long s_cnt[CNT_N];
     if (lane_id() < CNT_N) s_cnt[lane_id()] = 0ull;
     uint8_t *sc = a.scratch + (size_t)blockIdx.x * a.scratch_per_wave;
@@ -1301,8 +1307,8 @@
         const int t = next_work_item(a.work_counter);
         if (t >= a.b.n_reads) break;
         int rd = a.b.order[t];
-        if (a.manhattan) k1_read<true, true>(a, rd, sc, (lds_u8 *)s_arena, MTR_ARENA_INTS * 4, s_cnt);
-        else k1_read<false, true>(a, rd, sc, (lds_u8 *)s_arena, MTR_ARENA_INTS * 4, s_cnt);
+        if (a.manhattan) k1_read<true, true>(a, rd, sc, (lds_u8 *)s_arena, K1_ARENA_INTS * 4, s_cnt);
+        else k1_read<false, true>(a, rd, sc, (lds_u8 *)s_arena, K1_ARENA_INTS * 4, s_cnt);
         loop_join();
     }
     wc_flush(s_cnt, a.counters);
diff --git a/mtr_amd/csrc/k2_units.hip.inc b/mtr_amd/csrc/k2_units.hip.inc
--- a/mtr_amd/csrc/k2_units.hip.inc
+++ b/mtr_amd/csrc/k2_units.hip.inc
@@ -405,6 +405,11 @@
     return mx;
 }
 
+static_assert(MTRC_MAX_SEEDS <= 512, "the seeds beyond the LDS ones lie in the 512 words of y.pol_u");
+DEVINL int *seeds_global(const K2Ctx &c) { return (int *)(c.sc + c.y.pol_u); }
+DEVINL void seed_put(K2Ctx &c, int n, int key) { if (n < K2_SEEDS_LDS) c.seeds[n] = key; else seeds_global(c)[n] = key; }
+DEVINL int seed_get(const K2Ctx &c, int n) { return n < K2_SEEDS_LDS ? (int)c.seeds[n] : seeds_global(c)[n]; }
+
 DEVINL int tab_seeds(K2Ctx &c, int k, int qs, int qe, int max_freq)
 {
     const int lane = lane_id();
@@ -418,7 +423,7 @@
         while (m != 0ull && n < MTRC_MAX_SEEDS) {
             int t = first_lane(m);
             int sk = lane_val(key, t);
-            if (lane == 0) { c.seeds[n] = sk; tab_dec(c, sk); }
+            if (lane == 0) { seed_put(c, n, sk); tab_dec(c, sk); }
             n++;
             m &= ~__ballot(cand && key == sk);
             m &= ~(1ull << t);
@@ -504,6 +509,9 @@
     hi = uni(ends[bhi]);
 }
 
+#define K2_STAGE_IDX_BITS 12
+static_assert(4 * MTRC_MAX_TIEBREAKS <= (1 << K2_STAGE_IDX_BITS), "a scan index fits the low bits of a staged match");
+static_assert((long long)MTRC_MAX_SUPPORTED_LENGTH + 1 < (1ll << (32 - K2_STAGE_IDX_BITS)), "count + 1 of a k-mer (at most the read's positions) fits the bits above the scan index");
 DEVINL int lookahead(K2Ctx &c, bool backward, int node, int k, int look, int &m_exit, long long &lookups)
 {
     const int lane = lane_id();
@@ -630,7 +638,7 @@
                 const unsigned long long hm = __ballot(hit);
                 if (hm != 0ull) {
                     const int pos = nmatch + mbcnt(hm);
-                    if (hit && pos < 64) { c.stage[pos] = cnt; c.stage[64 + pos] = idx; c.stage[128 + pos] = d; }
+                    if (hit && pos < 64) c.stage[pos] = (int)(((unsigned)(cnt + 1) << K2_STAGE_IDX_BITS) | (unsigned)idx);
                     nmatch += __popcll(hm);
                 }
                 loop_join();
@@ -645,7 +653,16 @@
                 } else {
                     __builtin_amdgcn_wave_barrier();
                     const bool mine = lane < nmatch;
-                    const int cnt = mine ? c.stage[lane] : -1, idx = mine ? c.stage[64 + lane] : 0x7fffffff, d = mine ? c.stage[128 + lane] : 0;
+                    const unsigned pk = mine ? (unsigned)c.stage[lane] : 0u;
+                    const int cnt = (int)(pk >> K2_STAGE_IDX_BITS) - 1, idx = mine ? (int)(pk & ((1u << K2_STAGE_IDX_BITS) - 1u)) : 0x7fffffff;
+                    int d;
+                    {
+                        const int ti = idx >> 2, j = idx & 3, x = ti & emask;
+                        const int bv = __shfl(breg, (ti >> (2 * e)) & 63, 64);
+                        if (!backward) d = (bv << (2 * (e + 1))) | (x << 2) | j;
+                        else d = bv | (int)(rev_digits((unsigned)x, e) << (2 * m0)) | (j << (2 * (m0 + e)));
+                        if (!mine) d = 0;
+                    }
                     best = wave_max_i32_dpp(cnt);
                     const bool tie = mine && cnt == best;
                     int rank = 0;
@@ -655,9 +672,10 @@
                     }
                     const unsigned long long tm = __ballot(tie);
                     nf = __popcll(tm);
-                    if (tie) c.stage[192 + rank] = d;
                     __builtin_amdgcn_wave_barrier();
-                    best_digit = uni(c.stage[192]);
+                    if (tie) c.stage[rank] = d;
+                    __builtin_amdgcn_wave_barrier();
+                    best_digit = uni(c.stage[0]);
                 }
             }
         }
@@ -682,7 +700,7 @@
                 if (eq != 0ull) {
                     if (nf == 0) best_digit = lane_val(digit, first_lane(eq));
                     const int pos = nf + mbcnt(eq);
-                    if (cnt == best && ci < ncand && pos < MTRC_MAX_TIEBREAKS) { if (pos < 64) c.stage[192 + pos] = digit; else Bn[pos] = digit; }
+                    if (cnt == best && ci < ncand && pos < MTRC_MAX_TIEBREAKS) { if (pos < 64) c.stage[pos] = digit; else Bn[pos] = digit; }
                     nf += __popcll(eq); if (nf > MTRC_MAX_TIEBREAKS) nf = MTRC_MAX_TIEBREAKS;
                 }
                 loop_join();
@@ -695,7 +713,7 @@
         } else {
             __builtin_amdgcn_wave_barrier();
             nb = nf; e = 0; m0 = m;
-            breg = lane < nb ? c.stage[192 + lane] : 0;
+            breg = lane < nb ? c.stage[lane] : 0;
             if (nb > 64) { Bn[lane] = breg; wave_sync_mem(); int *sw = B; B = Bn; Bn = sw; }
         }
         loop_join();
@@ -920,7 +938,7 @@
     for (int b = s; b < ns && first == ns; b += 64) {
         const int idx = b + lane;
         const bool act = idx < ns;
-        const int sd = act ? (int)c.seeds[idx] : 0;
+        const int sd = act ? seed_get(c, idx) : 0;
         const int r = walk_screen(c.lds_keys, c.tab, k, sd, act ? 1 : 0, max_steps, backward ? 1 : 0);
         const unsigned long long m = __ballot(act && r != 0);
         if (m != 0ull) first = b + first_lane(m);
@@ -1241,7 +1259,7 @@
             const int dir = 1 - turn;
             if (turn == 1 && !found_bwd) break;
             for (int s = 0; s < ns; s++) {
-                int seed = uni(c.seeds[s]);
+                int seed = uni(seed_get(c, s));
                 int period = walk(c, dir == 1, qs, qe, k, seed, K2_NSLOT_FIXED + n_ent);
                 found = period > 0 ? 1 : 0;
                 if (!found && s + MTRC_SCREEN_MIN_SEEDS < ns) {
@@ -1269,10 +1287,18 @@
 }
 
 
-#define POL_OUT_OFF 512
-static_assert(MTRC_MAX_PERIOD <= POL_OUT_OFF, "a staged unit and its polished form share the look-ahead's staging bytes");
-DEVINL int pol_base(const lds_u8 *st, int j) { return uni((int)st[j]) & 3; }
-DEVINL int pol_score(const lds_u8 *st, int j) { return (uni((int)st[j]) >> 2) & 3; }
+#define POL_STAGE_POS (8 * K2_STAGE_INTS)
+static_assert(MTRC_MAX_PERIOD <= POL_STAGE_POS && POL_STAGE_POS == K2_SLOT_SCORE, "a staged unit fits the look-ahead's staging row");
+static_assert(1024 + MTRC_MAX_PERIOD <= 512 * 4, "the polished unit lies in the second KB of y.pol_u (the first holds seeds)");
+DEVINL uint8_t *pol_out(const K2Ctx &c) { return c.sc + c.y.pol_u + 1024; }
+DEVINL int pol_nib(const lds_u8 *st, int j) { return ((int)st[j >> 1] >> (4 * (j & 1))) & 15; }
+DEVINL void pol_stage_put(lds_u8 *st, int t, int v)
+{
+    const int hi = __shfl_down(v, 1, 64);
+    if ((t & 1) == 0) st[t >> 1] = (unsigned char)((v & 15) | ((hi & 15) << 4));
+}
+DEVINL int pol_base(const lds_u8 *st, int j) { return uni(pol_nib(st, j)) & 3; }
+DEVINL int pol_score(const lds_u8 *st, int j) { return (uni(pol_nib(st, j)) >> 2) & 3; }
 DEVINL void wave_sync_lds()
 {
     asm volatile("s_waitcnt lgkmcnt(0)" ::: "memory");
@@ -1283,7 +1309,7 @@
     DEVINL unsigned long long word(int q) const { return (unsigned long long)lane_val64(v, q); }
 };
 struct PolOps {
-    const K2Ctx *c; const lds_u8 *st; lds_u8 *out; int k, period;
+    const K2Ctx *c; const lds_u8 *st; uint8_t *out; int k, period;
     DEVINL int base(int j) const { return pol_base(st, j); }
     DEVINL int score(int j) const { return pol_score(st, j); }
     DEVINL int get(int node) const { return uni(tab_get(*c, node)); }
@@ -1304,19 +1330,19 @@
         const int lane = lane_id();
         const bool on = lane < 2 * k;
         int pos = j + (k - 1 - (lane >> 1)); if (pos >= period) pos -= period;
-        const int b = on ? (int)st[pos] : 0;
+        const int b = on ? pol_nib(st, pos) : 0;
         return (int)(unsigned)__ballot(on && ((b >> (lane & 1)) & 1) != 0);
     }
     DEVINL void emit(int jr, int b) const { if (lane_id() == 0) out[jr] = (unsigned char)b; }
     DEVINL void copy(int jr, int j, int n) const
     {
 #pragma unroll 1
-        for (int t = j - n + 1 + lane_id(); t <= j; t += 64) out[jr - j + t] = (unsigned char)(st[t] & 3);
+        for (int t = j - n + 1 + lane_id(); t <= j; t += 64) out[jr - j + t] = (unsigned char)(pol_nib(st, t) & 3);
     }
     DEVINL void undefined() const { wc_add(c->wc, CNT_UNDEFINED, 1); }
     DEVINL void join() const { loop_join(); }
 };
-DEVINL bool polish_staged(K2Ctx &c, const RR &r, const lds_u8 *st, lds_u8 *out, int &jr, unsigned long long t_stage)
+DEVINL bool polish_staged(K2Ctx &c, const RR &r, const lds_u8 *st, uint8_t *out, int &jr, unsigned long long t_stage)
 {
     const int lane = lane_id();
     const int k = r.kmer, period = r.period;
@@ -1325,7 +1351,7 @@
 #pragma unroll 1
     for (int q = 0; q * 64 < period; q++) {
         const int t = q * 64 + lane;
-        const unsigned long long w = __ballot(t < period && pp_flagged([&](int p) { return ((int)st[p] >> 2) & 3; }, k, t));
+        const unsigned long long w = __ballot(t < period && pp_flagged([&](int p) { return (pol_nib(st, p) >> 2) & 3; }, k, t));
         if (lane == q) m.v = (long long)w;
         any |= w;
     }
@@ -1343,7 +1369,7 @@
 #else
     const bool ok = pp_walk_plan(ops, m, k, period, jr, altered);
 #endif
-    wave_sync_lds();
+    wave_sync_mem();
     wc_time_pol(c.wc, CNT_SPARE47, t_walk);
     return ok && altered;
 }
@@ -1354,10 +1380,10 @@
     const int k = r.kmer, period = r.period;
     if (period <= k) return;
     uint8_t *ub = slot_unit(c, slot); const int *score = slot_score(c, slot);
-    lds_u8 *st = (lds_u8 *)c.stage, *out = st + POL_OUT_OFF;
+    lds_u8 *st = (lds_u8 *)c.stage; uint8_t *out = pol_out(c);
     const unsigned long long t_stage = clk();
 #pragma unroll 1
-    for (int t = lane; t < period; t += 64) st[t] = pp_stage_byte((int)ub[t], score[t]);
+    for (int t0 = 0; t0 < period; t0 += 64) { const int t = t0 + lane; pol_stage_put(st, t, t < period ? (int)pp_stage_byte((int)ub[t], score[t]) : 0); }
     wave_sync_lds();
     int jr = 0;
     if (!polish_staged(c, r, st, out, jr, t_stage)) return;
@@ -1736,10 +1762,10 @@
 template <bool MANHATTAN>
 __global__ __launch_bounds__(64, MTR_WAVES_PER_SIMD) void mtr_k_reads(K1Args a1, K2Args a)
 {
-    __shared__ __attribute__((aligned(16))) int s_arena[MTR_ARENA_INTS];
+    __shared__ __attribute__((aligned(16))) int s_arena[K1_ARENA_INTS];
     __shared__ unsigned long long s_cnt[CNT_N];
-    static_assert(MTR_ARENA_INTS == K2_TAB_CAP + MTRC_MAX_SEEDS + 4 + 4 * 64, "arena layout");
-    int *s_keys = s_arena, *s_seeds = s_arena + K2_TAB_CAP, *s_stage = s_seeds + MTRC_MAX_SEEDS + 4;
+    static_assert(MTR_ARENA_INTS == K2_TAB_CAP + K2_SEEDS_LDS + K2_STAGE_INTS && K1_ARENA_INTS >= MTR_ARENA_INTS, "arena layout");
+    int *s_keys = s_arena, *s_seeds = s_arena + K2_TAB_CAP, *s_stage = s_seeds + K2_SEEDS_LDS;
     if (lane_id() < CNT_N) s_cnt[lane_id()] = 0ull;
     K2Ctx c;
     c.a = &a;
@@ -1758,7 +1784,7 @@
 #ifdef MTR_PROFILE
         const unsigned long long rt_read = __builtin_amdgcn_s_memrealtime();
 #endif
-        k1_read<MANHATTAN>(a1, c.rd, c.sc, (lds_u8 *)s_arena, MTR_ARENA_INTS * 4, s_cnt);
+        k1_read<MANHATTAN>(a1, c.rd, c.sc, (lds_u8 *)s_arena, K1_ARENA_INTS * 4, s_cnt);
         wave_sync_mem();
         k2_read(c);
         wc_time(s_cnt, CYC_TOTAL, t_read);
@@ -1779,7 +1805,7 @@
 {
     __shared__ __attribute__((aligned(16))) int s_arena[MTR_ARENA_INTS];
     __shared__ unsigned long long s_cnt[CNT_N];
-    int *s_keys = s_arena, *s_seeds = s_arena + K2_TAB_CAP, *s_stage = s_seeds + MTRC_MAX_SEEDS + 4;
+    int *s_keys = s_arena, *s_seeds = s_arena + K2_TAB_CAP, *s_stage = s_seeds + K2_SEEDS_LDS;
     if (lane_id() < CNT_N) s_cnt[lane_id()] = 0ull;
     K2Ctx c;
     c.a = &a;
diff --git a/mtr_amd/csrc/k3_staged.hip.inc b/mtr_amd/csrc/k3_staged.hip.inc
--- a/mtr_amd/csrc/k3_staged.hip.inc
+++ b/mtr_amd/csrc/k3_staged.hip.inc
@@ -276,7 +276,7 @@
 }
 DEVINL void st_park_entries(K2Ctx &c, const StagedArgs &s, long long base, const RangeP1 &st, int min_k, int stride, int n_slots, int maxU)
 {
-    const int lane = lane_id();
+    const int lane = lane_here();
     const int *pmeta = (const int *)(c.sc + c.y.pool_meta);
     StEnt *en = (StEnt *)(s.arena + base + sizeof(StItemHdr));
     for (int e = 0; e < st.n_ent; e++) {
@@ -358,7 +358,7 @@
 {
     __shared__ __attribute__((aligned(16))) int s_arena[MTR_ARENA_INTS];
     __shared__ unsigned long long s_cnt[CNT_N];
-    int *s_keys = s_arena, *s_seeds = s_arena + K2_TAB_CAP, *s_stage = s_seeds + MTRC_MAX_SEEDS + 4;
+    int *s_keys = s_arena, *s_seeds = s_arena + K2_TAB_CAP, *s_stage = s_seeds + K2_SEEDS_LDS;
     const int lane = lane_id();
     if (lane < CNT_N) s_cnt[lane] = 0ull;
     K2Ctx c;
@@ -448,11 +448,14 @@
     wc_flush(s_cnt, a.counters);
 }
 
-__global__ __launch_bounds__(64, MTR_WAVES_PER_SIMD) void mtr_k_walks_k(K2Args a, StagedArgs s)
+#ifndef MTR_WALKS_K_WAVES_PER_SIMD
+#define MTR_WALKS_K_WAVES_PER_SIMD MTR_LAT_WAVES_PER_SIMD
+#endif
+__global__ __launch_bounds__(64, MTR_WALKS_K_WAVES_PER_SIMD) void mtr_k_walks_k(K2Args a, StagedArgs s)
 {
     __shared__ __attribute__((aligned(16))) int s_arena[MTR_ARENA_INTS];
     __shared__ unsigned long long s_cnt[CNT_N];
-    int *s_keys = s_arena, *s_seeds = s_arena + K2_TAB_CAP, *s_stage = s_seeds + MTRC_MAX_SEEDS + 4;
+    int *s_keys = s_arena, *s_seeds = s_arena + K2_TAB_CAP, *s_stage = s_seeds + K2_SEEDS_LDS;
     const int lane = lane_id();
     if (lane < CNT_N) s_cnt[lane] = 0ull;
     if (st_staged_overflowed(a)) return;
@@ -1019,7 +1022,7 @@
 {
     __shared__ __attribute__((aligned(16))) int s_arena[MTR_ARENA_INTS];
     __shared__ unsigned long long s_cnt[CNT_N];
-    int *s_keys = s_arena, *s_seeds = s_arena + K2_TAB_CAP, *s_stage = s_seeds + MTRC_MAX_SEEDS + 4;
+    int *s_keys = s_arena, *s_seeds = s_arena + K2_TAB_CAP, *s_stage = s_seeds + K2_SEEDS_LDS;
     const int lane = lane_id();
     if (lane < CNT_N) s_cnt[lane] = 0ull;
     if (st_staged_overflowed(a)) return;
@@ -1172,7 +1175,7 @@
 {
     __shared__ __attribute__((aligned(16))) int s_arena[MTR_ARENA_INTS];
     __shared__ unsigned long long s_cnt[CNT_N];
-    int *s_keys = s_arena, *s_seeds = s_arena + K2_TAB_CAP, *s_stage = s_seeds + MTRC_MAX_SEEDS + 4;
+    int *s_keys = s_arena, *s_seeds = s_arena + K2_TAB_CAP, *s_stage = s_seeds + K2_SEEDS_LDS;
     const int lane = lane_id();
     if (lane < CNT_N) s_cnt[lane] = 0ull;
     if (st_staged_overflowed(a)) return;
@@ -1228,7 +1231,7 @@
 {
     __shared__ __attribute__((aligned(16))) int s_arena[MTR_ARENA_INTS];
     __shared__ unsigned long long s_cnt[CNT_N];
-    int *s_keys = s_arena, *s_seeds = s_arena + K2_TAB_CAP, *s_stage = s_seeds + MTRC_MAX_SEEDS + 4;
+    int *s_keys = s_arena, *s_seeds = s_arena + K2_TAB_CAP, *s_stage = s_seeds + K2_SEEDS_LDS;
     const int lane = lane_id();
     if (lane < CNT_N) s_cnt[lane] = 0ull;
     if (st_staged_overflowed(a)) return;
@@ -1256,14 +1259,14 @@
         const unsigned long long t_in = clk();
         const int U = uni(en[e].period), maxU = st_max_unit(qs, qe);
         uint8_t *du = s.arena + ro + sizeof(StRev); int *ds = (int *)(s.arena + ro + sizeof(StRev) + K2_SLOT_UNIT);
-        lds_u8 *st = (lds_u8 *)c.stage, *out = st + POL_OUT_OFF;
+        lds_u8 *st = (lds_u8 *)c.stage; uint8_t *out = pol_out(c);
         {
             const uint8_t *su = st_slot_unit(s.arena, base, h, e); const int *ss = (const int *)(su + st_pad16(maxU));
             int sv[K2_SLOT_SCORE / 64]; int bv[K2_SLOT_SCORE / 64];
 #pragma unroll
             for (int q = 0; q < K2_SLOT_SCORE / 64; q++) { const int t = q * 64 + lane; sv[q] = t < U ? ss[t] : -1; bv[q] = t < U ? (int)su[t] : 0; }
 #pragma unroll
-            for (int q = 0; q < K2_SLOT_SCORE / 64; q++) { const int t = q * 64 + lane; ds[t] = sv[q]; if (t < POL_OUT_OFF) st[t] = pp_stage_byte(bv[q], sv[q]); }
+            for (int q = 0; q < K2_SLOT_SCORE / 64; q++) { const int t = q * 64 + lane; ds[t] = sv[q]; pol_stage_put(st, t, (int)pp_stage_byte(bv[q], sv[q])); }
         }
         wave_sync_lds();
         wc_time_pol(c.wc, CNT_SPARE44, t_in);
@@ -1277,11 +1280,12 @@
             const int np = (MTRC_MAX_PERIOD - 1) - jr;
 #pragma unroll 1
             for (int t = lane; t < np; t += 64) du[t] = out[t + jr + 1];
+            wave_sync_mem();
             cur.period = np;
             st_rr_store(rv->rr, cur);
         } else {
 #pragma unroll 1
-            for (int t = lane; t < U; t += 64) du[t] = (uint8_t)(st[t] & 3);
+            for (int t = lane; t < U; t += 64) du[t] = (uint8_t)(pol_nib(st, t) & 3);
         }
         if (trace_on(c, 4)) {
             wave_sync_mem();
@@ -1418,7 +1422,10 @@
 }
 #define MTR_RQ_LDS_BYTES (RQ_SLOTS * 64 + CNT_N * 8)
 static_assert(16 * MTR_ARENA_CORESIDENT_BYTES + 4 * MTR_LDS_ALLOC(MTR_RQ_LDS_BYTES) <= MTR_LDS_PER_CU, "four DP wavefronts beside sixteen arena wavefronts");
-static_assert(16 * MTR_LDS_ALLOC(MTR_ARENA_INTS * 4 + CNT_N * 8) <= MTR_LDS_PER_CU, "sixteen wavefronts of an arena kernel per CU");
+#ifndef MTR_ARENA_ANY_SIZE
+static_assert(MTR_ARENA_INTS * 4 + CNT_N * 8 <= MTR_ARENA_CORESIDENT_BYTES, "an arena kernel declares at most seven LDS granules");
+#endif
+static_assert(16 * MTR_LDS_ALLOC(K1_ARENA_INTS * 4 + CNT_N * 8) <= MTR_LDS_PER_CU, "sixteen wavefronts of an arena kernel per CU");
 __global__ __launch_bounds__(64, MTR_WAVES_PER_SIMD) void mtr_k_revise_quads(K2Args a, StagedArgs s)
 {
     typedef __attribute__((address_space(3))) StRevMember lds_StRevMember;
```

After: 308,500, median of 6. Within noise of the previous version (+0.9%).
